# kasirershahartau/tissue_image_processing

Hardware: AMD Instinct MI355X
Metric: frames/sec end-to-end (2048^2, z=30) (higher is better)
Workload: dtype f32(f16x3)

## Files before the change

tissue_image_processing_amd/csrc/tip_core.hip:

```cpp
#include "tip_internal.h"
#include <algorithm>
#include <cmath>
#include <cstdlib>
#include <map>
#include <mutex>

namespace tip {

static thread_local Ctx *g_ctx = nullptr;
static thread_local int g_requested_device = 0;

static int ctx_create(int device)
{
    Ctx *c = new Ctx();
    c->device = device;
    hipError_t e = hipSetDevice(device);
    if (e != hipSuccess) {
        c->err = std::string("hipSetDevice failed: ") + hipGetErrorString(e);
        g_ctx = c;
        return TIP_ERR_HIP;
    }
    {
        const char *pr = getenv("TIP_STREAM_PRIORITY");
        int lo = 0, hi = 0;
        if (pr && hipDeviceGetStreamPriorityRange(&lo, &hi) == hipSuccess && (strcmp(pr, "low") == 0 || strcmp(pr, "high") == 0))
            e = hipStreamCreateWithPriority(&c->stream, hipStreamNonBlocking, strcmp(pr, "low") == 0 ? lo : hi);
        else
            e = hipStreamCreateWithFlags(&c->stream, hipStreamNonBlocking);
    }
    if (e != hipSuccess) {
        c->err = std::string("hipStreamCreate failed: ") + hipGetErrorString(e);
        c->stream = nullptr;
        g_ctx = c;
        return TIP_ERR_HIP;
    }
    g_ctx = c;
    return TIP_OK;
}

Ctx &ctx()
{
    if (!g_ctx) ctx_create(g_requested_device);
    return *g_ctx;
}

int fail(int code, const char *fmt, ...)
{
    char buf[1024];
    va_list ap;
    va_start(ap, fmt);
    vsnprintf(buf, sizeof buf, fmt, ap);
    va_end(ap);
    ctx().err = buf;
    return code;
}

int launch_check(const char *what)
{
    hipError_t e = hipGetLastError();
    if (e != hipSuccess) return fail(TIP_ERR_HIP, "launch %s: %s", what, hipGetErrorString(e));
    return TIP_OK;
}

void *ws_alloc(size_t bytes)
{
    Ctx &c = ctx();
    bytes = (bytes + 255) & ~(size_t)255;
    int best = -1;
    for (size_t i = 0; i < c.pool.size(); i++)
        if (!c.pool[i].used && c.pool[i].bytes >= bytes && (best < 0 || c.pool[i].bytes < c.pool[best].bytes))
            best = (int)i;
    if (best >= 0 && c.pool[best].bytes <= 2 * bytes + (1 << 20)) {
        c.pool[best].used = true;
        return c.pool[best].p;
    }
    void *p = nullptr;
    hipError_t e = hipMalloc(&p, bytes);
    if (e != hipSuccess) {
        for (auto &b : c.pool)
            if (!b.used && b.p) { (void)hipFree(b.p); b.p = nullptr; b.bytes = 0; }
        e = hipMalloc(&p, bytes);
        if (e != hipSuccess) {
            fail(TIP_ERR_NOMEM, "hipMalloc(%zu) failed: %s", bytes, hipGetErrorString(e));
            return nullptr;
        }
    }
    c.pool.push_back({p, bytes, true});
    return p;
}

void *pinned_scratch(size_t bytes)
{
    Ctx &c = ctx();
    if (c.pin_bytes >= bytes && c.pin_buf) return c.pin_buf;
    if (c.pin_buf) { (void)hipHostFree(c.pin_buf); c.pin_buf = nullptr; c.pin_bytes = 0; }
    const size_t want = bytes + (bytes >> 2) + 4096;
    void *p = nullptr;
    if (hipHostMalloc(&p, want, hipHostMallocDefault) != hipSuccess) {
        (void)hipGetLastError();
        fail(TIP_ERR_NOMEM, "hipHostMalloc(%zu) failed", want);
        return nullptr;
    }
    c.pin_buf = p;
    c.pin_bytes = want;
    return p;
}

void ws_free(void *p)
{
    Ctx &c = ctx();
    for (auto &b : c.pool)
        if (b.p == p) { b.used = false; return; }
}

void prof_begin(const char *name)
{
    Ctx &c = ctx();
    if (!c.prof) return;
    ProfRec r;
    r.name = name;
    if (c.free_events.size() >= 2) {
        r.e0 = c.free_events.back(); c.free_events.pop_back();
        r.e1 = c.free_events.back(); c.free_events.pop_back();
    } else {
        (void)hipEventCreate(&r.e0);
        (void)hipEventCreate(&r.e1);
    }
    (void)hipEventRecord(r.e0, c.stream);
    c.recs.push_back(r);
}

void prof_end()
{
    Ctx &c = ctx();
    if (!c.prof) return;
    (void)hipEventRecord(c.recs.back().e1, c.stream);
}

namespace {
Tuning g_tuning;
std::once_flag g_tuning_once;
std::mutex g_tuning_mu;

bool tuning_assign(Tuning &t, const char *name, const char *value)
{
    const Tuning def;
    const bool unset = !value || !*value;
    auto flag = [&](int &field, int dflt) { field = unset ? dflt : (strcmp(value, "0") != 0 ? 1 : 0); };
    auto num = [&](int &field, int dflt) { field = unset ? dflt : atoi(value); };
    auto pair = [&](int &a, int &b, int da, int db) {
        a = da; b = db;
        if (!unset) sscanf(value, "%d,%d", &a, &b);
    };
    const std::string n(name ? name : "");
    if (n == "TIP_WS_TIES") {
        if (unset) t.ws_ties = def.ws_ties;
        else t.ws_ties = (!strcmp(value, "fast") || !strcmp(value, "0")) ? 0 : 1;
    }
    else if (n == "TIP_WS_OPEN") pair(t.ws_open_a, t.ws_open_b, def.ws_open_a, def.ws_open_b);
    else if (n == "TIP_WS_NO_SKIP") flag(t.ws_no_skip, 0);
    else if (n == "TIP_WS_DEBUG") flag(t.ws_debug, 0);
    else if (n == "TIP_WS_NO_ENDGAME") flag(t.ws_no_endgame, 0);
    else if (n == "TIP_WS_NO_WIDE") flag(t.ws_no_wide, 0);
    else if (n == "TIP_PROJECT_GENERIC") flag(t.project_generic, 0);
    else if (n == "TIP_PROJECT_UNFUSED_PREBLUR") flag(t.project_unfused_preblur, 0);
    else if (n == "TIP_PROJECT_UNFUSED_MASK") flag(t.project_unfused_mask, 0);
    else if (n == "TIP_PROJECT_EXACT_SCORE") flag(t.project_exact_score, 0);
    else if (n == "TIP_PROJECT_DEBUG") flag(t.project_debug, 0);
    else if (n == "TIP_UNET_TILE8") num(t.unet_tile8, def.unet_tile8);
    else if (n == "TIP_UF_ONE_LEVEL") flag(t.uf_one_level, 0);
    else if (n == "TIP_UNET_SPB") num(t.unet_spb, def.unet_spb);
    else if (n == "TIP_UNET_MFMA") { num(t.unet_mfma, def.unet_mfma); if (t.unet_mfma != 32) t.unet_mfma = 16; }
    else if (n == "TIP_UNET_XCD_MAP") flag(t.unet_xcd_map, 1);
    else if (n == "TIP_UNET_FIRST") {
        if (unset || !strcmp(value, "mfma")) t.unet_first_mfma = def.unet_first_mfma;
        else t.unet_first_mfma = !strcmp(value, "valu") ? 0 : std::max(atoi(value), 0);
    }
    else if (n == "TIP_UNET_TAIL_UNFUSED") flag(t.unet_tail_unfused, 0);
    else if (n == "TIP_MB_SMALL") num(t.mb_small, def.mb_small);
    else if (n == "TIP_MB_BATCH") num(t.mb_batch, def.mb_batch);
    else return false;
    return true;
}

const char *const TUNING_NAMES[] = {"TIP_WS_TIES", "TIP_WS_OPEN", "TIP_WS_NO_SKIP", "TIP_WS_DEBUG", "TIP_WS_NO_ENDGAME", "TIP_WS_NO_WIDE",
                                    "TIP_PROJECT_GENERIC", "TIP_PROJECT_UNFUSED_PREBLUR", "TIP_PROJECT_UNFUSED_MASK",
                                    "TIP_PROJECT_EXACT_SCORE", "TIP_PROJECT_DEBUG", "TIP_UNET_TILE8", "TIP_UNET_TAIL_UNFUSED", "TIP_UNET_XCD_MAP", "TIP_UNET_SPB", "TIP_UNET_MFMA", "TIP_UNET_FIRST", "TIP_UF_ONE_LEVEL", "TIP_MB_SMALL", "TIP_MB_BATCH"};

void tuning_from_env()
{
    for (const char *name : TUNING_NAMES)
        if (const char *e = getenv(name)) tuning_assign(g_tuning, name, e);
}
}

const Tuning &tuning()
{
    std::call_once(g_tuning_once, tuning_from_env);
    return g_tuning;
}

int make_taps(Taps &t, const double *w, int n)
{
    if (n <= 0 || n > 255 || !(n & 1)) return fail(TIP_ERR_ARG, "tap count %d must be odd and <= 255", n);
    for (int i = 1; i <= n / 2; i++)
        if (fabs(w[n / 2 + i] - w[n / 2 - i]) > 2.220446049250313e-16)
            return fail(TIP_ERR_UNSUPPORTED, "only symmetric kernels (scipy's symmetric correlate1d branch)");
    memset(&t, 0, sizeof t);
    for (int i = 0; i < n; i++) t.w[i] = w[i];
    t.n = n;
    return TIP_OK;
}

static double np_pairwise_sum(const double *a, long n)
{
    if (n < 8) {
        double r = 0.0;
        for (long i = 0; i < n; i++) r += a[i];
        return r;
    } else if (n <= 128) {
        double r[8];
        long i;
        for (i = 0; i < 8; i++) r[i] = a[i];
        for (i = 8; i < n - (n % 8); i += 8)
            for (int k = 0; k < 8; k++) r[k] += a[i + k];
        double res = ((r[0] + r[1]) + (r[2] + r[3])) + ((r[4] + r[5]) + (r[6] + r[7]));
        for (; i < n; i++) res += a[i];
        return res;
    }
    long n2 = n / 2;
    n2 -= n2 % 8;
    return np_pairwise_sum(a, n2) + np_pairwise_sum(a + n2, n - n2);
}

int libm_taps(double sigma, double truncate, double *w, int cap)
{
    long radius = (long)(truncate * sigma + 0.5);
    long n = 2 * radius + 1;
    if (n > cap) return -1;
    double s2 = sigma * sigma;
    for (long i = 0; i < n; i++) {
        double x = (double)(i - radius);
        w[i] = exp(-0.5 / s2 * (x * x));
    }
    double sum = np_pairwise_sum(w, n);
    for (long i = 0; i < n; i++) w[i] = w[i] / sum;
    return (int)n;
}

}

using namespace tip;

extern "C" {

int tip_version(void) { return 100; }

int tip_device_count(void)
{
    int n = 0;
    if (hipGetDeviceCount(&n) != hipSuccess) return 0;
    return n;
}

int tip_init(int device)
{
    if (g_ctx) {
        if (g_ctx->device == device && g_ctx->stream) return TIP_OK;
        tip_shutdown();
    }
    g_requested_device = device;
    int rc = ctx_create(device);
    return rc;
}

int tip_shutdown(void)
{
    if (!g_ctx) return TIP_OK;
    Ctx *c = g_ctx;
    if (c->stream) (void)hipStreamSynchronize(c->stream);
    for (auto &b : c->pool)
        if (b.p) (void)hipFree(b.p);
    for (auto &r : c->recs) { (void)hipEventDestroy(r.e0); (void)hipEventDestroy(r.e1); }
    for (auto &e : c->free_events) (void)hipEventDestroy(e);
    if (c->edge_event) (void)hipEventDestroy(c->edge_event);
    if (c->prep_ws) (void)hipFree(c->prep_ws);
    if (c->unet_status) (void)hipFree(c->unet_status);
    if (c->unet_status_host) (void)hipHostFree(c->unet_status_host);
    if (c->pin_buf) (void)hipHostFree(c->pin_buf);
    if (c->stream) (void)hipStreamDestroy(c->stream);
    delete c;
    g_ctx = nullptr;
    return TIP_OK;
}

int tip_last_error(char *buf, size_t n)
{
    if (!buf || !n) return TIP_ERR_ARG;
    const std::string &e = ctx().err;
    snprintf(buf, n, "%s", e.c_str());
    return TIP_OK;
}

int tip_malloc(void **dptr, size_t bytes)
{
    if (!dptr) return fail(TIP_ERR_ARG, "tip_malloc: null out pointer");
    Ctx &c = ctx();
    if (!c.stream) return TIP_ERR_HIP;
    TIP_HIP(hipMalloc(dptr, bytes ? bytes : 16));
    return TIP_OK;
}

int tip_free(void *dptr)
{
    if (!dptr) return TIP_OK;
    Ctx &c = ctx();
    if (c.stream) TIP_HIP(hipStreamSynchronize(c.stream));
    TIP_HIP(hipFree(dptr));
    return TIP_OK;
}

int tip_memcpy_h2d(void *dst, const void *src, size_t bytes)
{
    Ctx &c = ctx();
    if (!c.stream) return TIP_ERR_HIP;
    TIP_HIP(hipMemcpyAsync(dst, src, bytes, hipMemcpyHostToDevice, c.stream));
    TIP_HIP(hipStreamSynchronize(c.stream));
    return TIP_OK;
}

int tip_memcpy_d2h(void *dst, const void *src, size_t bytes)
{
    Ctx &c = ctx();
    if (!c.stream) return TIP_ERR_HIP;
    TIP_HIP(hipMemcpyAsync(dst, src, bytes, hipMemcpyDeviceToHost, c.stream));
    TIP_HIP(hipStreamSynchronize(c.stream));
    return TIP_OK;
}

int tip_memcpy_d2d(void *dst, const void *src, size_t bytes)
{
    Ctx &c = ctx();
    if (!c.stream) return TIP_ERR_HIP;
    prof_begin("memcpy_d2d");
    const hipError_t e = hipMemcpyAsync(dst, src, bytes, hipMemcpyDeviceToDevice, c.stream);
    prof_end();
    TIP_HIP(e);
    return TIP_OK;
}

int tip_memcpy2d_d2d(void *dst, size_t dst_pitch, const void *src, size_t src_pitch, size_t width_bytes, size_t height)
{
    Ctx &c = ctx();
    if (!c.stream) return TIP_ERR_HIP;
    if (!dst || !src || width_bytes > dst_pitch || width_bytes > src_pitch) return fail(TIP_ERR_ARG, "tip_memcpy2d_d2d: bad arguments");
    if (width_bytes == 0 || height == 0) return TIP_OK;
    TIP_HIP(hipMemcpy2DAsync(dst, dst_pitch, src, src_pitch, width_bytes, height, hipMemcpyDeviceToDevice, c.stream));
    return TIP_OK;
}

int tip_memset(void *dst, int value, size_t bytes)
{
    Ctx &c = ctx();
    if (!c.stream) return TIP_ERR_HIP;
    TIP_HIP(hipMemsetAsync(dst, value, bytes, c.stream));
    return TIP_OK;
}

int tip_sync(void)
{
    Ctx &c = ctx();
    if (!c.stream) return TIP_ERR_HIP;
    TIP_HIP(hipStreamSynchronize(c.stream));
    return TIP_OK;
}

int tip_pointer_device(const void *p)
{
    hipPointerAttribute_t a;
    if (!p || hipPointerGetAttributes(&a, p) != hipSuccess) { (void)hipGetLastError(); return TIP_ERR_ARG; }
    if (a.type != hipMemoryTypeDevice) return TIP_ERR_ARG;
    return a.device;
}

int tip_wait_stream(void *stream)
{
    Ctx &c = ctx();
    if (!c.stream) return TIP_ERR_HIP;
    if (!c.edge_event) TIP_HIP(hipEventCreateWithFlags(&c.edge_event, hipEventDisableTiming));
    TIP_HIP(hipEventRecord(c.edge_event, (hipStream_t)stream));
    TIP_HIP(hipStreamWaitEvent(c.stream, c.edge_event, 0));
    return TIP_OK;
}

int tip_stream_wait_tip(void *stream)
{
    Ctx &c = ctx();
    if (!c.stream) return TIP_ERR_HIP;
    if (!c.edge_event) TIP_HIP(hipEventCreateWithFlags(&c.edge_event, hipEventDisableTiming));
    TIP_HIP(hipEventRecord(c.edge_event, c.stream));
    TIP_HIP(hipStreamWaitEvent((hipStream_t)stream, c.edge_event, 0));
    return TIP_OK;
}

int tip_prof_enable(int on)
{
    ctx().prof = on != 0;
    return TIP_OK;
}

int tip_prof_reset(void)
{
    Ctx &c = ctx();
    if (c.stream) (void)hipStreamSynchronize(c.stream);
    for (auto &r : c.recs) { c.free_events.push_back(r.e0); c.free_events.push_back(r.e1); }
    c.recs.clear();
    return TIP_OK;
}

int tip_prof_report(char *buf, size_t n)
{
    Ctx &c = ctx();
    if (c.stream) (void)hipStreamSynchronize(c.stream);
    std::map<std::string, std::pair<long, double>> agg;
    std::vector<std::string> order;
    for (auto &r : c.recs) {
        float ms = 0.f;
        if (hipEventElapsedTime(&ms, r.e0, r.e1) != hipSuccess) ms = 0.f;
        auto it = agg.find(r.name);
        if (it == agg.end()) { agg[r.name] = {1, (double)ms}; order.push_back(r.name); }
        else { it->second.first++; it->second.second += ms; }
    }
    std::string s;
    char line[256];
    for (auto &k : order) {
        snprintf(line, sizeof line, "%s %ld %.6f\n", k.c_str(), agg[k].first, agg[k].second);
        s += line;
    }
    if (buf && n) snprintf(buf, n, "%s", s.c_str());
    return (int)s.size() + 1;
}

int tip_set_tuning(const char *name, const char *value)
{
    (void)tuning();
    std::lock_guard<std::mutex> lock(g_tuning_mu);
    if (!tuning_assign(g_tuning, name, value)) return fail(TIP_ERR_ARG, "tip_set_tuning: unknown name %s", name ? name : "(null)");
    return TIP_OK;
}

int tip_gaussian_taps(double sigma, double truncate, double *taps, int cap)
{
    if (!taps || sigma <= 0) return fail(TIP_ERR_ARG, "tip_gaussian_taps: bad arguments");
    int n = libm_taps(sigma, truncate, taps, cap);
    if (n < 0) return fail(TIP_ERR_OVERFLOW, "tip_gaussian_taps: capacity %d too small", cap);
    return n;
}

}
```

tissue_image_processing_amd/csrc/tip_corr.h:

```cpp
#pragma once
#include "tip_internal.h"
#include <type_traits>

namespace tip {

template <typename T>
struct LoadPlain {
    const T *p;
    long sz, sy;
    __device__ __forceinline__ double operator()(int z, int y, int x) const { return (double)p[z * sz + y * sy + x]; }
};

__device__ __forceinline__ int clampi(int v, int lo, int hi) { return v < lo ? lo : (v > hi ? hi : v); }

template <int R, typename At, typename W>
__device__ __forceinline__ double tap_sum(At at, const W &w)
{
    double tmp = at(R) * w[R];
#pragma unroll
    for (int d = R; d >= 1; --d) tmp += (at(R - d) + at(R + d)) * w[R - d];
    return tmp;
}
template <typename At, typename W>
__device__ __forceinline__ double tap_sum(int r, At at, const W &w)
{
    double tmp = at(r) * w[r];
    for (int d = r; d >= 1; --d) tmp += (at(r - d) + at(r + d)) * w[r - d];
    return tmp;
}

struct TapsDev {
    const double *w;
    int n;
};

template <int FIRST = 0, typename F>
static inline int with_axis(int axis, F &&f)
{
    if constexpr (FIRST == 0)
        if (axis == 0) return f(std::integral_constant<int, 0>{});
    if (axis == 1) return f(std::integral_constant<int, 1>{});
    return f(std::integral_constant<int, 2>{});
}

template <typename T, int AXIS, typename Load, typename TapSrc = Taps>
__global__ void __launch_bounds__(256) k_corr_generic(Load in, T *__restrict__ out, int Z, int Y, int X, TapSrc taps)
{
    const int x = blockIdx.x * blockDim.x + threadIdx.x;
    const int y = blockIdx.y;
    const int z = blockIdx.z;
    if (x >= X) return;
    const int r = taps.n >> 1;
    const int len = AXIS == 0 ? Z : (AXIS == 1 ? Y : X);
    const int c = AXIS == 0 ? z : (AXIS == 1 ? y : x);
    auto at = [&](int j) -> double {
        const int i = clampi(c - r + j, 0, len - 1);
        return AXIS == 0 ? in(i, y, x) : (AXIS == 1 ? in(z, i, x) : in(z, y, i));
    };
    out[((long)z * Y + y) * X + x] = (T)tap_sum(r, at, taps.w);
}

template <int AXIS, int NW>
__device__ __forceinline__ void stage_tile(float *tile, const float *__restrict__ src, int npos, int first, int l0, int Y, int X,
                                           int lane, int wave)
{
    constexpr int LS = AXIS == 1 ? 64 : 65;
    if (AXIS == 1) {
        constexpr int UL = 8;
        const int xx = min(l0 + lane, X - 1);
        for (int pb = wave; pb < npos; pb += NW * UL) {
            float v[UL];
#pragma unroll
            for (int u = 0; u < UL; ++u) v[u] = src[(long)clampi(first + pb + u * NW, 0, Y - 1) * X + xx];
#pragma unroll
            for (int u = 0; u < UL; ++u)
                if (pb + u * NW < npos) tile[(pb + u * NW) * LS + lane] = v[u];
        }
    } else {
        for (int l = wave; l < 64; l += 2 * NW) {
            float v[2][8];
#pragma unroll
            for (int h = 0; h < 2; ++h) {
                const int yy = min(l0 + l + h * NW, Y - 1);
#pragma unroll
                for (int u = 0; u < 8; ++u) v[h][u] = src[(long)yy * X + clampi(first + lane + 64 * u, 0, X - 1)];
            }
#pragma unroll
            for (int h = 0; h < 2; ++h)
#pragma unroll
                for (int u = 0; u < 8; ++u)
                    if (lane + 64 * u < npos && l + h * NW < 64) tile[(lane + 64 * u) * LS + l + h * NW] = v[h][u];
        }
    }
}

template <int AXIS, int TO, int R>
__global__ void __launch_bounds__(256) k_corr_long_f32(const float *__restrict__ in, float *__restrict__ out,
                                                       int Z, int Y, int X, Taps taps)
{
    extern __shared__ __attribute__((aligned(16))) float tile[];
    constexpr int LS = AXIS == 1 ? 64 : 65;
    const int r = taps.n >> 1;
    const int npos = TO + 2 * r;
    const int lane = threadIdx.x & 63;
    const int wave = threadIdx.x >> 6;
    const int z = blockIdx.z;
    const int len = AXIS == 1 ? Y : X;
    const int nlines = AXIS == 1 ? X : Y;
    const int p0 = blockIdx.y * TO;
    const int l0 = blockIdx.x * 64;
    const float *src = in + (long)z * Y * X;
    float *dst = out + (long)z * Y * X;

    stage_tile<AXIS, 4>(tile, src, npos, p0 - r, l0, Y, X, lane, wave);
    __syncthreads();

    const int line = l0 + lane;
    constexpr int PER_WAVE = TO / 4;
    for (int g = 0; g < PER_WAVE / R; ++g) {
        const int o0 = wave * PER_WAVE + g * R;
        if (p0 + o0 >= len) break;
        const float *ctr = tile + (r + o0) * LS + lane;
        double acc[R], L[R], Rr[R];
        const double wc = taps.w[r];
#pragma unroll
        for (int i = 0; i < R; ++i) {
            acc[i] = (double)ctr[i * LS] * wc;
            L[i] = (double)ctr[(i - r) * LS];
            Rr[i] = (double)ctr[(i + r) * LS];
        }
#pragma unroll 8
        for (int d = r; d >= 1; --d) {
            const double w = taps.w[r - d];
#pragma unroll
            for (int i = 0; i < R; ++i) acc[i] += (L[i] + Rr[i]) * w;
#pragma unroll
            for (int i = 0; i < R - 1; ++i) L[i] = L[i + 1];
            L[R - 1] = (double)ctr[(R - 1 - (d - 1)) * LS];
#pragma unroll
            for (int i = R - 1; i > 0; --i) Rr[i] = Rr[i - 1];
            Rr[0] = (double)ctr[(d - 1) * LS];
        }
        if (line < nlines) {
            if (AXIS == 1) {
#pragma unroll
                for (int i = 0; i < R; ++i) {
                    const int yy = p0 + o0 + i;
                    if (yy < Y) dst[(long)yy * X + line] = (float)acc[i];
                }
            } else {
#pragma unroll
                for (int i = 0; i < R; ++i) {
                    const int xx = p0 + o0 + i;
                    if (xx < X) dst[(long)line * X + xx] = (float)acc[i];
                }
            }
        }
    }
}

}
```

tissue_image_processing_amd/csrc/tip_corr_f16.h:

```cpp
#pragma once
#include "tip_corr.h"
#include "tip_unet_conv.h"

namespace tip {

constexpr int HF_TO = 256, HF_LN = 32, HF_NW = 4;
typedef float hf_f32x4 __attribute__((ext_vector_type(4)));

struct HfScale {
    float s, inv;
};
__device__ __forceinline__ HfScale hf_scale(const float *clip_p95, const int *clip_has)
{
    const float c = (clip_has && *clip_has && *clip_p95 > 0.f) ? *clip_p95 : 1.f;
    const int e = min(max((int)((__float_as_uint(c) >> 23) & 0xffu) - 127, -60), 100);
    HfScale h;
    h.s = __uint_as_float((unsigned)(127 + 13 - e) << 23);
    h.inv = __uint_as_float((unsigned)(127 - 13 + e - 17) << 23);
    return h;
}

template <int AXIS, int R8>
__global__ void __launch_bounds__(HF_NW * 64, 2) k_corr_long_f16(const float *__restrict__ in, float *__restrict__ out, int Z, int Y, int X,
                                                                  TapsF taps, const float *__restrict__ clip_p95, const int *__restrict__ clip_has,
                                                                  int *__restrict__ range_flag, int tiles_ln, int tiles_pos, int xcd_bands)
{
    constexpr int r = 8 * R8, NPOS = HF_TO + 2 * r, S = R8 + 2;
    constexpr int PCH = (NPOS / 8) | 1, PITCH = PCH * 8;
    constexpr int WROWS = 2 * S + 3;
    extern __shared__ __attribute__((aligned(16))) unsigned char hf_smem[];
    _Float16 *sB_hi = reinterpret_cast<_Float16 *>(hf_smem), *sB_lo = sB_hi + HF_LN * PITCH;
    uint4 *sW_hi = reinterpret_cast<uint4 *>(sB_lo + HF_LN * PITCH), *sW_lo = sW_hi + WROWS * 8;
    const int tid = threadIdx.x, lane = tid & 63, wave = __builtin_amdgcn_readfirstlane(tid >> 6);
    const int z = blockIdx.y;
    int lx, py;
    if (AXIS == 2 && xcd_bands) {
        const int b = blockIdx.x, k = b & 7, j = b >> 3;
        py = j % tiles_pos;
        lx = k + 8 * (j / tiles_pos);
    } else {
        lx = blockIdx.x % tiles_ln;
        py = blockIdx.x / tiles_ln;
    }
    const int p0 = py * HF_TO, l0 = lx * HF_LN;
    const long P = (long)Y * X;
    const float *src = in + (long)z * P;
    const HfScale sc = hf_scale(clip_p95, clip_has);

    for (int idx = tid; idx < WROWS * 8; idx += HF_NW * 64) {
        const int up = (idx >> 3) - 3, c = idx & 7;
        f16x8 hi, lo;
#pragma unroll
        for (int e = 0; e < 8; ++e) {
            const int d = 8 * up - c + e, ad = d - r < 0 ? r - d : d - r;
            const float w = (d >= 0 && d <= 2 * r) ? taps.w[r - ad] * 131072.f : 0.f;
            hi[e] = (_Float16)w;
            lo[e] = (_Float16)((w - (float)hi[e]) * 2048.f);
        }
        sW_hi[idx] = __builtin_bit_cast(uint4, hi);
        sW_lo[idx] = __builtin_bit_cast(uint4, lo);
    }
    float vmax = 0.f;
    auto split8 = [&](const float (&v)[8], int line, int g) {
        f16x8 hi, lo;
#pragma unroll
        for (int e = 0; e < 8; ++e) {
            const float vs = v[e] * sc.s;
            vmax = fmax_raw(vmax, vs);
            hi[e] = (_Float16)vs;
            lo[e] = (_Float16)__builtin_fmaf(vs - (float)hi[e], 2048.f, fminf(vs * 1.329227995784916e36f, 5.9604644775390625e-8f));
        }
        *reinterpret_cast<uint4 *>(sB_hi + line * PITCH + 8 * g) = __builtin_bit_cast(uint4, hi);
        *reinterpret_cast<uint4 *>(sB_lo + line * PITCH + 8 * g) = __builtin_bit_cast(uint4, lo);
    };
    constexpr int NG = NPOS / 8;
    if (AXIS == 2) {
        constexpr int NIT = (HF_LN * NG + HF_NW * 64 - 1) / (HF_NW * 64);
        hf_f32x4 ld[NIT][2];
        const bool vec = (X & 3) == 0;
        constexpr int DL = (HF_NW * 64) / NG, DG = (HF_NW * 64) - DL * NG;
        const int line_0 = tid / NG, g_0 = tid - line_0 * NG;
        int uline[NIT], ug[NIT];
        {
            int line = line_0, g = g_0;
#pragma unroll
            for (int it = 0; it < NIT; ++it) {
                uline[it] = line;
                ug[it] = g;
                line += DL;
                g += DG;
                if (g >= NG) { g -= NG; ++line; }
            }
        }
#pragma unroll
        for (int it = 0; it < NIT; ++it) {
            const int line = uline[it], g = ug[it];
            const float *row = src + (long)min(l0 + min(line, HF_LN - 1), Y - 1) * X;
            const int x0 = p0 - r + 8 * g;
            if (vec && x0 >= 0 && x0 + 8 <= X) {
                ld[it][0] = *reinterpret_cast<const hf_f32x4 *>(row + x0);
                ld[it][1] = *reinterpret_cast<const hf_f32x4 *>(row + x0 + 4);
            } else {
                ld[it][0] = hf_f32x4{row[clampi(x0, 0, X - 1)], row[clampi(x0 + 1, 0, X - 1)], row[clampi(x0 + 2, 0, X - 1)], row[clampi(x0 + 3, 0, X - 1)]};
                ld[it][1] = hf_f32x4{row[clampi(x0 + 4, 0, X - 1)], row[clampi(x0 + 5, 0, X - 1)], row[clampi(x0 + 6, 0, X - 1)], row[clampi(x0 + 7, 0, X - 1)]};
            }
        }
#pragma unroll
        for (int it = 0; it < NIT; ++it) {
            const int line = uline[it], g = ug[it];
            if (line < HF_LN) {
                const float v[8] = {ld[it][0][0], ld[it][0][1], ld[it][0][2], ld[it][0][3], ld[it][1][0], ld[it][1][1], ld[it][1][2], ld[it][1][3]};
                split8(v, line, g);
            }
        }
    } else {
        constexpr int NIT = (NG * (HF_LN / 4) + HF_NW * 64 - 1) / (HF_NW * 64);
        hf_f32x4 ld[NIT][8];
        const int lq = tid & 7;
        const int xq = l0 + 4 * lq;
        const bool vec = (X & 3) == 0 && xq + 4 <= X;
        if (vec) {
#pragma unroll
            for (int it = 0; it < NIT; ++it) {
                const int g = min(it * (HF_NW * 8) + (tid >> 3), NG - 1), y0 = p0 - r + 8 * g;
#pragma unroll
                for (int e = 0; e < 8; ++e) ld[it][e] = *reinterpret_cast<const hf_f32x4 *>(src + (long)clampi(y0 + e, 0, Y - 1) * X + xq);
            }
        } else {
#pragma unroll
            for (int it = 0; it < NIT; ++it) {
                const int g = min(it * (HF_NW * 8) + (tid >> 3), NG - 1), y0 = p0 - r + 8 * g;
#pragma unroll
                for (int e = 0; e < 8; ++e) {
                    const float *row = src + (long)clampi(y0 + e, 0, Y - 1) * X;
                    ld[it][e] = hf_f32x4{row[min(xq, X - 1)], row[min(xq + 1, X - 1)], row[min(xq + 2, X - 1)], row[min(xq + 3, X - 1)]};
                }
            }
        }
#pragma unroll
        for (int it = 0; it < NIT; ++it) {
            const int g = it * (HF_NW * 8) + (tid >> 3);
            if (g < NG) {
                float v[8];
#pragma unroll
                for (int e = 0; e < 8; ++e) v[e] = ld[it][e].x;
                split8(v, 4 * lq, g);
#pragma unroll
                for (int e = 0; e < 8; ++e) v[e] = ld[it][e].y;
                split8(v, 4 * lq + 1, g);
#pragma unroll
                for (int e = 0; e < 8; ++e) v[e] = ld[it][e].z;
                split8(v, 4 * lq + 2, g);
#pragma unroll
                for (int e = 0; e < 8; ++e) v[e] = ld[it][e].w;
                split8(v, 4 * lq + 3, g);
            }
        }
    }
    if (!(vmax < 40000.f)) atomicOr(range_flag, 8);
    __syncthreads();

    const int i = lane & 31, h = lane >> 5;
    const int len = AXIS == 1 ? Y : X;
    if (p0 + wave * 64 >= len) return;
    const _Float16 *bh = sB_hi + i * PITCH + wave * 64 + 8 * h, *bl = sB_lo + i * PITCH + wave * 64 + 8 * h;
    const int wrow0 = (h - (i >> 3) + 3) * 8 + (i & 7);
    f32x16 thh[2], tm[2], ahh[2], am[2];
#pragma unroll
    for (int t = 0; t < 2; ++t)
#pragma unroll
        for (int q = 0; q < 16; ++q) { thh[t][q] = 0.f; tm[t][q] = 0.f; ahh[t][q] = 0.f; am[t][q] = 0.f; }
    uint4 fh[3], fl[3];
    auto mm = [](const uint4 &wf, const uint4 &sf, const f32x16 &c) -> f32x16 {
        if (AXIS == 1) return __builtin_amdgcn_mfma_f32_32x32x16_f16(__builtin_bit_cast(f16x8, wf), __builtin_bit_cast(f16x8, sf), c, 0, 0, 0);
        return __builtin_amdgcn_mfma_f32_32x32x16_f16(__builtin_bit_cast(f16x8, sf), __builtin_bit_cast(f16x8, wf), c, 0, 0, 0);
    };
    auto flush = [&](int t) {
#pragma unroll
        for (int q = 0; q < 16; q += 2) {
            f32x2 x = f32x2{thh[t][q], thh[t][q + 1]} + f32x2{ahh[t][q], ahh[t][q + 1]};
            f32x2 y = f32x2{tm[t][q], tm[t][q + 1]} + f32x2{am[t][q], am[t][q + 1]};
            asm volatile("" : "+v"(x), "+v"(y));
            thh[t][q] = x[0]; thh[t][q + 1] = x[1];
            tm[t][q] = y[0]; tm[t][q + 1] = y[1];
            ahh[t][q] = 0.f; ahh[t][q + 1] = 0.f;
            am[t][q] = 0.f; am[t][q + 1] = 0.f;
        }
    };
#pragma unroll
    for (int s = 0; s < S + 2; ++s) {
        const uint4 sh = *reinterpret_cast<const uint4 *>(bh + 16 * s), sl = *reinterpret_cast<const uint4 *>(bl + 16 * s);
        if (s < S) {
            fh[s % 3] = sW_hi[wrow0 + 16 * s];
            fl[s % 3] = sW_lo[wrow0 + 16 * s];
            ahh[0] = mm(fh[s % 3], sh, ahh[0]);
            am[0] = mm(fh[s % 3], sl, am[0]);
            am[0] = mm(fl[s % 3], sh, am[0]);
            if ((s & 1) == 1 || s == S - 1) flush(0);
        }
        if (s >= 2) {
            const int k = (s - 2) % 3;
            ahh[1] = mm(fh[k], sh, ahh[1]);
            am[1] = mm(fh[k], sl, am[1]);
            am[1] = mm(fl[k], sh, am[1]);
            if (((s - 2) & 1) == 1 || s == S + 1) flush(1);
        }
        __builtin_amdgcn_sched_barrier(0);
    }
    float *dst = out + (long)z * P;
#pragma unroll
    for (int t = 0; t < 2; ++t) {
        const int o0 = p0 + wave * 64 + 32 * t;
#pragma unroll
        for (int q = 0; q < 16; ++q) {
            const int rr = (q & 3) + 8 * (q >> 2) + 4 * h;
            const float val = __builtin_fmaf(tm[t][q], 4.8828125e-4f, thh[t][q]) * sc.inv;
            if (AXIS == 1) {
                const int yy = o0 + rr, xx = l0 + i;
                if (yy < Y && xx < X) dst[(long)yy * X + xx] = val;
            } else {
                const int yy = l0 + rr, xx = o0 + i;
                if (yy < Y && xx < X) dst[(long)yy * X + xx] = val;
            }
        }
    }
}

}
```

tissue_image_processing_amd/csrc/tip_internal.h:

```cpp
#pragma once
#include <hip/hip_runtime.h>
#include <cstdarg>
#include <cstdint>
#include <cstdio>
#include <cstring>
#include <string>
#include <vector>
#include "../../include/tissue_hip.h"

namespace tip {

struct ProfRec { const char *name; hipEvent_t e0, e1; };

struct Ctx {
    int device = -1;
    hipStream_t stream = nullptr;
    std::string err;
    struct Block { void *p; size_t bytes; bool used; };
    std::vector<Block> pool;
    int last_ws_labels = 0;
    long last_ws_other = 0;
    hipEvent_t edge_event = nullptr;
    void *prep_ws = nullptr;
    unsigned *unet_status = nullptr;
    int *unet_status_host = nullptr;
    void *pin_buf = nullptr;
    size_t pin_bytes = 0;
    bool prof = false;
    std::vector<ProfRec> recs;
    std::vector<hipEvent_t> free_events;
};

Ctx &ctx();
int fail(int code, const char *fmt, ...);
int launch_check(const char *what);
void *ws_alloc(size_t bytes);
void *pinned_scratch(size_t bytes);
void ws_free(void *p);

struct WsGuard {
    std::vector<void *> ptrs;
    template <typename T> T *get(size_t count) {
        void *p = ws_alloc(count * sizeof(T) ? count * sizeof(T) : 16);
        if (p) ptrs.push_back(p);
        return (T *)p;
    }
    ~WsGuard() { for (void *p : ptrs) ws_free(p); }
};

struct Staging {
    WsGuard ws;
    int rc = TIP_OK;
    struct Out { void *host; const void *dev; size_t bytes; };
    std::vector<Out> outs;

    bool hip(hipError_t e, const char *what)
    {
        if (e != hipSuccess && !rc) rc = fail(TIP_ERR_HIP, "%s failed: %s", what, hipGetErrorString(e));
        return !rc;
    }
    template <typename T> T *scratch(size_t count)
    {
        if (rc) return nullptr;
        T *d = ws.get<T>(count);
        if (!d) rc = TIP_ERR_NOMEM;
        return d;
    }
    template <typename T> T *in(const T *host, size_t count)
    {
        T *d = host ? scratch<T>(count) : nullptr;
        if (d && count) hip(hipMemcpyAsync(d, host, count * sizeof(T), hipMemcpyHostToDevice, ctx().stream), "hipMemcpyAsync (upload)");
        return d;
    }
    template <typename T> T *out(T *host, size_t count, bool zero = false)
    {
        T *d = host ? scratch<T>(count) : nullptr;
        if (d && zero && count) hip(hipMemsetAsync(d, 0, count * sizeof(T), ctx().stream), "hipMemsetAsync");
        if (d) outs.push_back({host, d, count * sizeof(T)});
        return d;
    }
    template <typename T> void set_count(const T *dev, size_t count)
    {
        for (Out &o : outs)
            if (o.dev == dev && count * sizeof(T) < o.bytes) o.bytes = count * sizeof(T);
    }
    int finish()
    {
        for (const Out &o : outs)
            if (o.bytes && !hip(hipMemcpyAsync(o.host, o.dev, o.bytes, hipMemcpyDeviceToHost, ctx().stream), "hipMemcpyAsync (download)")) break;
        if (!rc) hip(hipStreamSynchronize(ctx().stream), "hipStreamSynchronize");
        return rc;
    }
};

void prof_begin(const char *name);
void prof_end();

struct Tuning {
    int ws_ties = 1;
    int ws_open_a = -1, ws_open_b = -1;
    int ws_no_skip = 0;
    int ws_debug = 0;
    int ws_no_endgame = 0, ws_no_wide = 0;
    int project_generic = 0, project_unfused_preblur = 0, project_unfused_mask = 0;
    int project_exact_score = 0, project_debug = 0;
    int unet_tail_unfused = 0;
    int unet_xcd_map = 1;
    int unet_spb = 3;
    int unet_mfma = 32;
    int unet_first_mfma = 1;
    int uf_one_level = 0;
    int mb_small = -1;
    int mb_batch = -1;
    int unet_tile8 = -1;
};
const Tuning &tuning();

#define TIP_HIP(call)                                                                             \
    do {                                                                                          \
        hipError_t e__ = (call);                                                                  \
        if (e__ != hipSuccess)                                                                    \
            return tip::fail(TIP_ERR_HIP, "%s failed: %s (%s:%d)", #call, hipGetErrorString(e__), \
                             __FILE__, __LINE__);                                                 \
    } while (0)

#define TIP_LAUNCH(name, kernel, grid, block, shmem, ...)                                  \
    do {                                                                                   \
        tip::prof_begin(name);                                                             \
        hipLaunchKernelGGL(kernel, grid, block, shmem, tip::ctx().stream, __VA_ARGS__);    \
        tip::prof_end();                                                                   \
        hipError_t e__ = hipGetLastError();                                                \
        if (e__ != hipSuccess)                                                             \
            return tip::fail(TIP_ERR_HIP, "launch %s: %s", name, hipGetErrorString(e__));  \
    } while (0)

static inline int cdiv(long a, long b) { return (int)((a + b - 1) / b); }

struct Taps {
    double w[256];
    int n;
};
struct TapsF {
    float w[256];
    int n;
};

int make_taps(Taps &t, const double *w, int n);
int libm_taps(double sigma, double truncate, double *w, int cap);
int correlate1d_dev(const void *in, void *out, int dtype, int Z, int Y, int X, int axis, const Taps &t, int force);

constexpr int OF_F64_AS_U16 = 5;
int optical_flow_tvl1_dev(const void *ref, const void *mov, int dtype, int y, int x, float attachment, float tightness,
                          int num_warp, int num_iter, double tol, float *flow_out, int32_t *warps_host, int cap);

int exclusive_scan_i32(const int *in, int *out, long n, int *total_dev);
int scan_i32_dev(const int32_t *in, int32_t *out, int n);

int regionprops_dev(const int32_t *labels, const double *intensity, int Y, int X, int n, int64_t *area, int64_t *bbox4, int64_t *sumy,
                    int64_t *sumx, int64_t *pc3, double *isum);
int order_stats_dev(const int32_t *labels, const double *img, long n, int nlab, long long *rank, const long long *rank0, double *lo,
                    double *hi);
int gaussian3d_dev(const void *in, void *out, int dtype, int Z, int Y, int X, const double *tz, int nz, const double *ty, int ny,
                   const double *tx, int nx);
int rankfilter2d_dev(const void *in, void *out, int dtype, int Y, int X, int ky, int kx, int fp, int border, int is_max);
int watershed_dev(const double *img, int32_t *labels, int Y, int X, int wsl, int32_t *flags_host);

template <typename Key, typename F>
__device__ __forceinline__ void wave_combine(bool active, Key key, F f)
{
    unsigned long long todo = __ballot(active);
    const int lane = threadIdx.x & 63;
    while (todo) {
        const int leader = __ffsll((long long)todo) - 1;
        const Key lk = __shfl(key, leader, 64);
        const unsigned long long same = __ballot(active && key == lk) & todo;
        if (lane == leader) f(lk, __popcll(same));
        todo &= ~same;
    }
}

}
```

tissue_image_processing_amd/csrc/tip_project.hip:

```cpp
#include "tip_slide.h"
#include "tip_preblur.h"
#include "tip_corr.h"
#include "tip_corr_f16.h"
#include "tip_manifold.h"
#include "tip_project_binned.h"
#include <algorithm>
#include <atomic>
#include <cstdlib>

namespace tip {

struct ClipInfo {
    double p95d;
    float p95;
    int has;
};

template <typename T>
__device__ __forceinline__ T wave_inclusive_scan(T v, int lane)
{
    for (int d = 1; d < 64; d <<= 1) {
        const T o = __shfl_up(v, d, 64);
        if (lane >= d) v += o;
    }
    return v;
}

constexpr int HIST_PER_BLOCK = 57344;
__device__ __forceinline__ void hist_clear(unsigned int *h)
{
    for (int i = threadIdx.x; i < 32768; i += 1024) h[i] = 0;
    __syncthreads();
}
__device__ __forceinline__ void hist_bump(unsigned int *h, int val) { atomicAdd(&h[val >> 1], 1u << (16 * (val & 1))); }
__device__ __forceinline__ void hist_flush_all(const unsigned int *h, unsigned long long *__restrict__ hist)
{
    for (int i = threadIdx.x; i < 32768; i += 1024) {
        const unsigned int c = h[i];
        if (c & 0xffffu) atomicAdd(&hist[2 * i], (unsigned long long)(c & 0xffffu));
        if (c >> 16) atomicAdd(&hist[2 * i + 1], (unsigned long long)(c >> 16));
    }
}

__global__ void __launch_bounds__(1024) k_hist_u16(const uint16_t *__restrict__ in, long n, int airy,
                                                   unsigned long long *__restrict__ hist)
{
    __shared__ unsigned int h[32768];
    hist_clear(h);
    const long nchunks = (n + HIST_PER_BLOCK - 1) / HIST_PER_BLOCK;
    for (long chunk = blockIdx.x; chunk < nchunks; chunk += gridDim.x) {
        const long base = chunk * HIST_PER_BLOCK;
        constexpr int TRIPS = HIST_PER_BLOCK / (1024 * 8);
        if (base + HIST_PER_BLOCK <= n && ((((uintptr_t)(in + base)) & 15) == 0)) {
            uint4 v[TRIPS];
#pragma unroll
            for (int k = 0; k < TRIPS; ++k) v[k] = *reinterpret_cast<const uint4 *>(in + base + ((long)k * 1024 + threadIdx.x) * 8);
#pragma unroll
            for (int k = 0; k < TRIPS; ++k) {
                const unsigned int w[4] = {v[k].x, v[k].y, v[k].z, v[k].w};
#pragma unroll
                for (int j = 0; j < 4; ++j) {
#pragma unroll
                    for (int s = 0; s < 2; ++s) hist_bump(h, airy_offset((int)((w[j] >> (16 * s)) & 0xffffu), airy));
                }
            }
        } else {
            for (int k = 0; k < TRIPS; ++k) {
                const long i0 = base + ((long)k * 1024 + threadIdx.x) * 8;
                for (int j = 0; j < 8; ++j)
                    if (i0 + j < n) hist_bump(h, airy_offset((int)in[i0 + j], airy));
            }
        }
        __syncthreads();
        if (chunk + gridDim.x < nchunks) {
            for (int i = threadIdx.x; i < 32768; i += 1024) {
                unsigned int c = h[i];
                if ((c & 0xffffu) >= 8192u) { atomicAdd(&hist[2 * i], (unsigned long long)(c & 0xffffu)); c &= 0xffff0000u; h[i] = c; }
                if ((c >> 16) >= 8192u) { atomicAdd(&hist[2 * i + 1], (unsigned long long)(c >> 16)); h[i] = c & 0xffffu; }
            }
            __syncthreads();
        }
    }
    hist_flush_all(h, hist);
}

__global__ void __launch_bounds__(1024) k_hist_u16_box(const uint16_t *__restrict__ in, int Y, int X, int z0, int y0, int x0, int bz,
                                                       int by, int bx, int airy, unsigned long long *__restrict__ hist)
{
    __shared__ unsigned int h[32768];
    hist_clear(h);
    const long n = (long)bz * by * bx;
    const long base = (long)blockIdx.x * HIST_PER_BLOCK;
    for (int k = 0; k < HIST_PER_BLOCK / 1024; ++k) {
        const long i = base + (long)k * 1024 + threadIdx.x;
        if (i < n) {
            const int x = (int)(i % bx), y = (int)((i / bx) % by), z = (int)(i / ((long)bx * by));
            hist_bump(h, airy_offset((int)in[((long)(z0 + z) * Y + (y0 + y)) * X + (x0 + x)], airy));
        }
    }
    __syncthreads();
    hist_flush_all(h, hist);
}

__global__ void __launch_bounds__(1024) k_percentile95(const unsigned long long *__restrict__ hist, ClipInfo *out, int with_zero)
{
    __shared__ unsigned long long wave_tot[16];
    __shared__ unsigned long long s_n;
    __shared__ int s_chunk[2];
    __shared__ unsigned long long s_before[2];
    __shared__ int s_val[2];
    const int t = threadIdx.x, lane = t & 63, wave = t >> 6;
    unsigned long long s = 0;
    for (int b = t * 64; b < t * 64 + 64; ++b)
        if (b > 0 || with_zero) s += hist[b];
    unsigned long long inc = wave_inclusive_scan(s, lane);
    if (lane == 63) wave_tot[wave] = inc;
    __syncthreads();
    unsigned long long base = 0;
    for (int w = 0; w < wave; ++w) base += wave_tot[w];
    inc += base;
    if (t == 1023) s_n = inc;
    __syncthreads();
    const unsigned long long n = s_n;
    if (n == 0) {
        if (t == 0) { out->has = 0; out->p95 = 0.f; out->p95d = 0.0; }
        return;
    }
    const double quant = 95.0 / 100.0;
    const double virt = (double)(n - 1) * quant;
    const double fl = floor(virt);
    const double gamma = virt - fl;
    long long prev = (long long)fl;
    if (prev < 0) prev = 0;
    if (prev > (long long)n - 1) prev = (long long)n - 1;
    long long next = prev + 1;
    if (next > (long long)n - 1) next = (long long)n - 1;
    const unsigned long long exc = inc - s;
    if (s > 0) {
        if (exc <= (unsigned long long)prev && (unsigned long long)prev < inc) { s_chunk[0] = t; s_before[0] = exc; }
        if (exc <= (unsigned long long)next && (unsigned long long)next < inc) { s_chunk[1] = t; s_before[1] = exc; }
    }
    __syncthreads();
    if (wave < 2) {
        const unsigned long long k = (unsigned long long)(wave == 0 ? prev : next) - s_before[wave];
        const int b = s_chunk[wave] * 64 + lane;
        const unsigned long long ci = wave_inclusive_scan((b > 0 || with_zero) ? hist[b] : 0ULL, lane);
        const unsigned long long hit = __ballot(ci > k);
        if (lane == 0) s_val[wave] = hit ? s_chunk[wave] * 64 + (__ffsll((long long)hit) - 1) : 65535;
    }
    __syncthreads();
    if (t != 0) return;
    const float lo = (float)s_val[0], hi = (float)s_val[1];
    const double diff = (double)(hi - lo);
    double res = (double)lo + diff * gamma;
    if (gamma >= 0.5) res = (double)hi - diff * (1.0 - gamma);
    out->p95d = res;
    out->p95 = (float)res;
    out->has = 1;
}

struct LoadU16Clip {
    const uint16_t *p;
    long sz, sy;
    int airy;
    const ClipInfo *clip;
    __device__ __forceinline__ double operator()(int z, int y, int x) const
    {
        return (double)raw_sample(p[z * sz + y * sy + x], airy, clip->has != 0, clip->p95);
    }
};

__device__ __forceinline__ void emit_zmaps(long p, int plane, int Z, int min_z, int atoh_shift, int32_t *__restrict__ zsel,
                                           int32_t *__restrict__ zsel_atoh, int64_t *__restrict__ zmap, int *__restrict__ err)
{
    const int cz = min_z + plane;
    if (zmap) zmap[p] = cz;
    int ca = cz;
    if (atoh_shift != 0) {
        ca = cz + atoh_shift;
        ca = ca < 0 ? 0 : (ca > Z ? Z : ca);
    }
    if (cz >= Z || ca >= Z) {
        atomicOr(err, 1);
        zsel[p] = cz >= Z ? Z - 1 : cz;
        zsel_atoh[p] = ca >= Z ? Z - 1 : ca;
        return;
    }
    zsel[p] = cz;
    zsel_atoh[p] = ca;
}

__global__ void __launch_bounds__(256) k_argmax_z(const float *__restrict__ score, int Z, long P, int min_z,
                                                  int atoh_shift, int32_t *__restrict__ zsel,
                                                  int32_t *__restrict__ zsel_atoh, int64_t *__restrict__ zmap,
                                                  int *__restrict__ err)
{
    const long p = (long)blockIdx.x * blockDim.x + threadIdx.x;
    if (p >= P) return;
    float best = score[p];
    int bi = 0;
    for (int z = 1; z < Z; ++z) {
        const float s = score[(long)z * P + p];
        if (s > best) { best = s; bi = z; }
    }
    emit_zmaps(p, bi, Z, min_z, atoh_shift, zsel, zsel_atoh, zmap, err);
}

__global__ void k_identity(float *out, int n)
{
    const int i = blockIdx.x * blockDim.x + threadIdx.x;
    if (i < n * n) out[i] = (i / n == i % n) ? 1.f : 0.f;
}

struct LoadMaskTable {
    const float *T;
    const int32_t *zsel;
    int Zs;
    long X;
    __device__ __forceinline__ double operator()(int z, int y, int x) const
    {
        return (double)T[z * Zs + zsel[(long)y * X + x]];
    }
};

template <int MAXC>
__global__ void __launch_bounds__(256) k_xpass_wmax(const float *__restrict__ ymask, const uint16_t *__restrict__ img,
                                                    int C, int Zfull, int zlo, int Zs, int Y, int X, int airy,
                                                    unsigned chan_mask, Taps taps, double *__restrict__ proj)
{
    const int x = blockIdx.x * blockDim.x + threadIdx.x;
    const int y = blockIdx.y;
    if (x >= X) return;
    const int r = taps.n >> 1;
    const long P = (long)Y * X;
    float mx[MAXC];
#pragma unroll
    for (int c = 0; c < MAXC; ++c) mx[c] = 0.f;
    for (int z = 0; z < Zs; ++z) {
        const float *row = ymask + (long)z * P + (long)y * X;
        const float m = (float)tap_sum(r, [&](int j) { return (double)row[clampi(x - r + j, 0, X - 1)]; }, taps.w);
#pragma unroll
        for (int c = 0; c < MAXC; ++c) {
            if (c < C && ((chan_mask >> c) & 1u)) {
                const float v = airy_offset((float)img[((long)c * Zfull + zlo + z) * P + (long)y * X + x], airy);
                const float pr = v * m;
                mx[c] = z == 0 ? pr : (pr > mx[c] ? pr : mx[c]);
            }
        }
    }
#pragma unroll
    for (int c = 0; c < MAXC; ++c)
        if (c < C && ((chan_mask >> c) & 1u)) proj[(long)c * P + (long)y * X + x] = (double)mx[c];
}

constexpr int MASK_R = 8, MASK_W = 2 * MASK_R + 1, MASK_ZR = 4;
constexpr int FT_Y = 16, FT_X = 128, FT_W = FT_X + 2 * MASK_R, FT_H = FT_Y + 2 * MASK_R;
template <int MAXC>
__global__ void __launch_bounds__(256) k_mask_wmax_fused(const float *__restrict__ table, const int32_t *__restrict__ zsel,
                                                         const uint16_t *__restrict__ img, int C, int Zfull, int zlo, int Zs, int Y,
                                                         int X, int airy, unsigned chan_mask, Taps taps, double *__restrict__ proj)
{
    extern __shared__ float sT[];
    __shared__ unsigned char zs[FT_H][FT_W];
    __shared__ unsigned char cmin[FT_Y][FT_W], cmax[FT_Y][FT_W];
    __shared__ __attribute__((aligned(16))) float ybuf[2][FT_Y][FT_W];
    __shared__ int s_lo, s_hi;
    const int t = threadIdx.x;
    const int x0 = blockIdx.x * FT_X, y0 = blockIdx.y * FT_Y;
    const long P = (long)Y * X;
    for (int i = t; i < Zs * Zs; i += 256) sT[i] = table[i];
    for (int i = t; i < FT_H * FT_W; i += 256) {
        const int r = i / FT_W, c = i - r * FT_W;
        zs[r][c] = (unsigned char)zsel[(long)clampi(y0 - MASK_R + r, 0, Y - 1) * X + clampi(x0 - MASK_R + c, 0, X - 1)];
    }
    if (t == 0) { s_lo = Zs; s_hi = -1; }
    __syncthreads();
    int lo = Zs, hi = -1;
    for (int i = t; i < FT_Y * FT_W; i += 256) {
        const int r = i / FT_W, c = i - r * FT_W;
        int a = zs[r][c], b = a;
#pragma unroll
        for (int k = 1; k < MASK_W; ++k) { const int v = zs[r + k][c]; a = min(a, v); b = max(b, v); }
        cmin[r][c] = (unsigned char)a; cmax[r][c] = (unsigned char)b;
        lo = min(lo, a); hi = max(hi, b);
    }
    for (int d = 32; d >= 1; d >>= 1) { lo = min(lo, __shfl_xor(lo, d, 64)); hi = max(hi, __shfl_xor(hi, d, 64)); }
    if ((t & 63) == 0) { atomicMin(&s_lo, lo); atomicMax(&s_hi, hi); }
    __syncthreads();
    const int zaB = max(s_lo - MASK_ZR, 0), zbB = min(s_hi + MASK_ZR, Zs - 1);
    const int ty = t >> 4, cx = (t & 15) * 8;
    const int gy = y0 + ty, gx = x0 + cx;
    const bool live = gy < Y && gx < X;
    int za = Zs, zb = -1;
    if (live) {
        for (int c = cx; c < cx + 8 + 2 * MASK_R; ++c) { za = min(za, (int)cmin[ty][c]); zb = max(zb, (int)cmax[ty][c]); }
        za = max(za - MASK_ZR, 0); zb = min(zb + MASK_ZR, Zs - 1);
    }
    float mx[MAXC][8];
#pragma unroll
    for (int c = 0; c < MAXC; ++c)
#pragma unroll
        for (int k = 0; k < 8; ++k) mx[c][k] = 0.f;
    for (int z = zaB; z <= zbB; ++z) {
        float(*yb)[FT_W] = ybuf[(z - zaB) & 1];
        const float *Tz = sT + z * Zs;
        for (int i = t; i < FT_Y * FT_W; i += 256) {
            const int r = i / FT_W, c = i - r * FT_W;
            float val = 0.f;
            if (z >= (int)cmin[r][c] - MASK_ZR && z <= (int)cmax[r][c] + MASK_ZR)
                val = (float)tap_sum<MASK_R>([&](int j) { return (double)Tz[zs[r + j][c]]; }, taps.w);
            yb[r][c] = val;
        }
        __syncthreads();
        if (live && z >= za && z <= zb) {
            float v[8 + 2 * MASK_R];
#pragma unroll
            for (int i = 0; i < (8 + 2 * MASK_R) / 4; ++i) {
                const float4 f = *reinterpret_cast<const float4 *>(&yb[ty][cx + 4 * i]);
                v[4 * i] = f.x; v[4 * i + 1] = f.y; v[4 * i + 2] = f.z; v[4 * i + 3] = f.w;
            }
            float m[8];
#pragma unroll
            for (int k = 0; k < 8; ++k) m[k] = (float)tap_sum<MASK_R>([&](int j) { return (double)v[k + j]; }, taps.w);
#pragma unroll
            for (int c = 0; c < MAXC; ++c) {
                if (c < C && ((chan_mask >> c) & 1u)) {
                    const uint16_t *ip = img + ((long)c * Zfull + zlo + z) * P + (long)gy * X + gx;
                    unsigned short pix[8];
                    if (gx + 8 <= X && (X & 7) == 0) {
                        const uint4 u = *reinterpret_cast<const uint4 *>(ip);
                        pix[0] = u.x & 0xffff; pix[1] = u.x >> 16; pix[2] = u.y & 0xffff; pix[3] = u.y >> 16;
                        pix[4] = u.z & 0xffff; pix[5] = u.z >> 16; pix[6] = u.w & 0xffff; pix[7] = u.w >> 16;
                    } else {
#pragma unroll
                        for (int k = 0; k < 8; ++k) pix[k] = gx + k < X ? ip[k] : 0;
                    }
#pragma unroll
                    for (int k = 0; k < 8; ++k) {
                        const float pr = airy_offset((float)pix[k], airy) * m[k];
                        mx[c][k] = pr > mx[c][k] ? pr : mx[c][k];
                    }
                }
            }
        }
    }
    if (live) {
#pragma unroll
        for (int c = 0; c < MAXC; ++c)
            if (c < C && ((chan_mask >> c) & 1u))
#pragma unroll
                for (int k = 0; k < 8; ++k)
                    if (gx + k < X) proj[(long)c * P + (long)gy * X + gx + k] = (double)mx[c][k];
    }
}

static int cu_count()
{
    static int cus = 0;
    if (!cus) {
        hipDeviceProp_t prop;
        cus = hipGetDeviceProperties(&prop, ctx().device) == hipSuccess && prop.multiProcessorCount > 0 ? prop.multiProcessorCount : 256;
    }
    return cus;
}

static TapsF taps_f32(const double *w, int n)
{
    TapsF f;
    f.n = n;
    for (int i = 0; i < 256; ++i) f.w[i] = i < n ? (float)w[i] : 0.f;
    return f;
}

template <int AXIS>
static int launch_f16(const float *in, float *out, int Zs, int Y, int X, const TapsF &t, const ClipInfo *clip, int *range_flag)
{
    if (t.n != 241 || !clip || !range_flag) return fail(TIP_ERR_ARG, "f16 score pass: %d taps (241 only) or no clip value / range flag", t.n);
    constexpr int R8 = 15, NPOS = HF_TO + 16 * R8, PITCH = ((NPOS / 8) | 1) * 8, WROWS = 2 * (R8 + 2) + 3;
    const size_t lds = (size_t)2 * HF_LN * PITCH * 2 + (size_t)2 * WROWS * 8 * 16;
    auto k = k_corr_long_f16<AXIS, R8>;
    static std::atomic<unsigned> attr_done[64];
    const int dev = ctx().device >= 0 && ctx().device < 64 ? ctx().device : 0;
    if (!(attr_done[dev].load(std::memory_order_acquire) & (1u << AXIS))) {
        TIP_HIP(hipFuncSetAttribute((const void *)k, hipFuncAttributeMaxDynamicSharedMemorySize, (int)lds));
        attr_done[dev].fetch_or(1u << AXIS, std::memory_order_release);
    }
    const int tiles_ln = cdiv(AXIS == 1 ? X : Y, HF_LN), tiles_pos = cdiv(AXIS == 1 ? Y : X, HF_TO);
    if ((long)tiles_ln * tiles_pos > 0x7fffffffL || Zs > 65535) return fail(TIP_ERR_ARG, "f16 score pass: grid too large");
    const dim3 grid((unsigned)(tiles_ln * tiles_pos), (unsigned)Zs);
    const int xcd_bands = (AXIS == 2 && tiles_ln % 8 == 0) ? 1 : 0;
    TIP_LAUNCH(AXIS == 1 ? "score_fast_y" : "score_fast_x", k, grid, dim3(HF_NW * 64), lds, in, out, Zs, Y, X, t, &clip->p95, &clip->has, range_flag,
               tiles_ln, tiles_pos, xcd_bands);
    return TIP_OK;
}

#define CERT_EPS (96.0f * 5.9604644775390625e-8f)
__device__ __forceinline__ float cert_abs(const ClipInfo *clip)
{
    return (clip && clip->has) ? clip->p95 * 5.684341886080802e-14f + 1e-30f : 1e-30f;
}

__global__ void __launch_bounds__(256) k_argmax_certify(const float *__restrict__ score, int Z, long P, int *__restrict__ best_z,
                                                        int *__restrict__ unc_list, int *__restrict__ unc_count, const ClipInfo *clip)
{
    __shared__ int s_cnt[4], s_base;
    const float dabs = cert_abs(clip);
    const long p0 = ((long)blockIdx.x * blockDim.x + threadIdx.x) * 4;
    const bool vec = p0 + 4 <= P && (P & 3) == 0;
    float b1[4], b2[4];
    int z1[4];
#pragma unroll
    for (int k = 0; k < 4; ++k) { b1[k] = -1.f; b2[k] = -1.f; z1[k] = 0; }
    if (p0 < P) {
        for (int z = 0; z < Z; ++z) {
            float v[4];
            if (vec) {
                const float4 f = *reinterpret_cast<const float4 *>(score + (long)z * P + p0);
                v[0] = f.x; v[1] = f.y; v[2] = f.z; v[3] = f.w;
            } else {
#pragma unroll
                for (int k = 0; k < 4; ++k) v[k] = p0 + k < P ? score[(long)z * P + p0 + k] : 0.f;
            }
#pragma unroll
            for (int k = 0; k < 4; ++k) {
                if (v[k] > b1[k]) { b2[k] = b1[k]; b1[k] = v[k]; z1[k] = z; }
                else if (v[k] > b2[k]) b2[k] = v[k];
            }
        }
    }
    unsigned unc = 0;
#pragma unroll
    for (int k = 0; k < 4; ++k) {
        if (p0 + k >= P) continue;
        best_z[p0 + k] = z1[k];
        const bool certain = (b1[k] == 0.f) || (Z == 1) || (b1[k] * (1.f - CERT_EPS) - dabs > b2[k] * (1.f + CERT_EPS) + dabs);
        if (!certain) unc |= 1u << k;
    }
    const int mine = __popc(unc);
    const int lane = threadIdx.x & 63, wave = threadIdx.x >> 6;
    const int incl = wave_inclusive_scan(mine, lane);
    if (lane == 63) s_cnt[wave] = incl;
    __syncthreads();
    if (threadIdx.x == 0) {
        const int tot = s_cnt[0] + s_cnt[1] + s_cnt[2] + s_cnt[3];
        s_base = tot ? atomicAdd(unc_count, tot) : 0;
    }
    __syncthreads();
    if (mine) {
        int off = s_base + incl - mine;
        for (int w = 0; w < wave; ++w) off += s_cnt[w];
#pragma unroll
        for (int k = 0; k < 4; ++k)
            if ((unc >> k) & 1u) unc_list[off++] = (int)(p0 + k);
    }
}

constexpr int FIX_UL = 16;
__global__ void __launch_bounds__(256) k_argmax_exact_fix(const float *__restrict__ zvol, const float *__restrict__ score, int Z, int Y,
                                                          int X, Taps taps, const int *__restrict__ unc_list,
                                                          const int *__restrict__ unc_count, int *__restrict__ best_z, const ClipInfo *clip)
{
    const float dabs = cert_abs(clip);
    __shared__ float c[256];
    __shared__ float sfast[64];
    __shared__ float sexact[64];
    __shared__ int s_z;
    const int r = taps.n >> 1;
    const int total = *unc_count, xcd = blockIdx.x & 7, per = (total + 7) / 8;
    for (int sl = blockIdx.x >> 3; sl < per; sl += gridDim.x >> 3) {
        const int u = xcd * per + sl;
        if (u >= total) break;
        const int p = unc_list[u];
        const int y = p / X, x = p - y * X;
        const long P = (long)Y * X;
        if (threadIdx.x < Z) sfast[threadIdx.x] = score[(long)threadIdx.x * P + p];
        __syncthreads();
        float smax = sfast[0];
        for (int z = 1; z < Z; ++z) smax = fmaxf(smax, sfast[z]);
        const float thr = smax * (1.f - CERT_EPS) - dabs;
        for (int z = 0; z < Z; ++z) {
            const bool cand = sfast[z] * (1.f + CERT_EPS) + dabs >= thr;
            if (!cand) { if (threadIdx.x == 0) sexact[z] = -1.f; continue; }
            const float *vol = zvol + (long)z * P;
            if (threadIdx.x < 2 * r + 1) {
                const int xx = clampi(x + (int)threadIdx.x - r, 0, X - 1);
                double tmp = (double)vol[(long)y * X + xx] * taps.w[r];
                for (int d0 = r; d0 >= 1; d0 -= FIX_UL) {
                    float a[FIX_UL], b[FIX_UL];
#pragma unroll
                    for (int u = 0; u < FIX_UL; ++u) {
                        const int d = max(d0 - u, 1);
                        a[u] = vol[(long)clampi(y - d, 0, Y - 1) * X + xx];
                        b[u] = vol[(long)clampi(y + d, 0, Y - 1) * X + xx];
                    }
#pragma unroll
                    for (int u = 0; u < FIX_UL; ++u)
                        if (d0 - u >= 1) tmp += ((double)a[u] + (double)b[u]) * taps.w[r - (d0 - u)];
                }
                c[threadIdx.x] = (float)tmp;
            }
            __syncthreads();
            if (threadIdx.x == 0) sexact[z] = (float)tap_sum(r, [&](int j) { return (double)c[j]; }, taps.w);
            __syncthreads();
        }
        if (threadIdx.x == 0) {
            float b = -2.f; int bz = 0;
            for (int z = 0; z < Z; ++z)
                if (sexact[z] > b) { b = sexact[z]; bz = z; }
            best_z[p] = bz;
        }
        __syncthreads();
    }
}

__global__ void __launch_bounds__(256) k_emit_zmaps(const int *__restrict__ best_z, int Z, long P, int min_z, int atoh_shift,
                                                    int32_t *__restrict__ zsel, int32_t *__restrict__ zsel_atoh,
                                                    int64_t *__restrict__ zmap, int *__restrict__ err)
{
    const long p = (long)blockIdx.x * blockDim.x + threadIdx.x;
    if (p >= P) return;
    emit_zmaps(p, best_z[p], Z, min_z, atoh_shift, zsel, zsel_atoh, zmap, err);
}

static int resolve_taps(const double *given, double sigma, int expect, Taps &t)
{
    double buf[256];
    if (!given) {
        int n = libm_taps(sigma, 4.0, buf, 255);
        if (n != expect) return fail(TIP_ERR_ARG, "internal: tap count %d != %d", n, expect);
        given = buf;
    }
    return make_taps(t, given, expect);
}

static int manifold_dev(const float *score, int Zs, int Y, int X, int *bestz, int *err)
{
    Ctx &c = ctx();
    const long P = (long)Y * X, V = (long)Zs * P;
    if (V >= 0xffffffffL || Zs > 144 || Zs < 1) return fail(TIP_ERR_UNSUPPORTED, "build_manifold: stack too large");
    WsGuard ws;
    unsigned long long *key = ws.get<unsigned long long>(1);
    if (!key) return TIP_ERR_NOMEM;
    TIP_HIP(hipMemsetAsync(key, 0, sizeof(unsigned long long), c.stream));
    TIP_HIP(hipMemsetAsync(bestz, 0xff, P * sizeof(int), c.stream));
    TIP_LAUNCH("argmax_first", k_argmax_first_f32, dim3((unsigned)std::min<long>(1024, cdiv(V, 256))), dim3(256), 0, score, V, key);
    int chunk = 1024;
    while (chunk > 64 && (size_t)4 * Zs * chunk > 150000) chunk >>= 1;
    const size_t lds = (size_t)4 * Zs * chunk;
    TIP_HIP(hipFuncSetAttribute((const void *)k_manifold, hipFuncAttributeMaxDynamicSharedMemorySize, (int)lds));
    TIP_LAUNCH("manifold", k_manifold, dim3(1), dim3(MAN_T), lds, score, Zs, Y, X, (const unsigned long long *)key, (volatile int *)bestz,
               chunk, err);
    return TIP_OK;
}

struct ProjJob {
    const uint16_t *czyx, *ref;
    int C, Z, Y, X, zlo, Zs;
    long P, V;
    int min_z, ref_ch, method, bin, airyscan, atoh_shift;
    bool manifold;
    bool ref_unshifted;
    bool fast;
    Taps k05, k1, k2, k30;
    WsGuard ws;
    float *A, *B;
    unsigned long long *hist;
    ClipInfo *clip;
    int32_t *zsel, *zsel_a;
    float *ident, *table;
    int *err;
    double *proj;
    int64_t *zmap;
    hipStream_t stream;
};

static int check_args(const ProjJob &s, int zhi, bool tile)
{
    if (!s.czyx || !s.proj) return fail(TIP_ERR_ARG, "project: null pointer");
    if (s.C < 1 || s.C > 8) return fail(TIP_ERR_ARG, "project: 1..8 channels supported (got %d)", s.C);
    if (s.ref_ch < 0 || s.ref_ch >= s.C) return fail(TIP_ERR_INDEX, "project: reference_channel %d out of range", s.ref_ch);
    if (s.zlo < 0 || zhi > s.Z || zhi <= s.zlo) return fail(TIP_ERR_ARG, "project: bad z range [%d,%d) of %d", s.zlo, zhi, s.Z);
    if (s.Y < 1 || s.X < 1 || s.Y > 65535) return fail(TIP_ERR_ARG, "project: bad frame size %dx%d", s.Y, s.X);
    if (s.manifold && tile) return fail(TIP_ERR_UNSUPPORTED, "project: build_manifold takes whole frames");
    if (s.manifold && (s.V >= 0xffffffffL || s.Zs > 144)) return fail(TIP_ERR_UNSUPPORTED, "project: build_manifold: stack too large");
    return TIP_OK;
}

static int take_workspace(ProjJob &s)
{
    s.A = s.ws.get<float>(s.V), s.B = s.ws.get<float>(s.V);
    s.hist = s.ws.get<unsigned long long>(65536);
    s.clip = s.ws.get<ClipInfo>(1);
    s.zsel = s.ws.get<int32_t>(s.P), s.zsel_a = s.ws.get<int32_t>(s.P);
    s.ident = s.ws.get<float>((size_t)s.Zs * s.Zs), s.table = s.ws.get<float>((size_t)s.Zs * s.Zs);
    s.err = s.ws.get<int>(1);
    if (!s.A || !s.B || !s.hist || !s.clip || !s.zsel || !s.zsel_a || !s.ident || !s.table || !s.err) return TIP_ERR_NOMEM;
    return TIP_OK;
}

static int clip_of_channel(ProjJob &s, const uint16_t *src, int with_zero, ClipInfo *clip)
{
    TIP_HIP(hipMemsetAsync(s.hist, 0, 65536 * sizeof(unsigned long long), s.stream));
    TIP_LAUNCH("hist_u16", k_hist_u16, dim3((unsigned)std::min<long>(cdiv(s.V, HIST_PER_BLOCK), cu_count())), dim3(1024), 0, src, s.V,
               s.airyscan, s.hist);
    TIP_LAUNCH("percentile95", k_percentile95, dim3(1), dim3(1024), 0, (const unsigned long long *)s.hist, clip, with_zero);
    return TIP_OK;
}

static int short_blur(ProjJob &s, const uint16_t *src, ClipInfo *ci)
{
    const int Zs = s.Zs, Y = s.Y, X = s.X;
    if (s.fast && s.bin == 1 && !tuning().project_unfused_preblur) {
        ShortTaps s05, s1;
        for (int i = 0; i < 8; ++i) { s05.w[i] = i < 3 ? s.k05.w[i] : 0.0; s1.w[i] = i < 5 ? s.k1.w[i] : 0.0; }
        TIP_LAUNCH("preblur_fused", k_preblur_fused, dim3(cdiv(X, PB_X), cdiv(Y, PB_Y)), dim3(PB_T), 0, src, s.airyscan,
                   (const float *)&ci->p95, (const int *)&ci->has, s.B, Zs, Y, X, s05, s1);
        return TIP_OK;
    }
    if (s.fast) {
        Src4U16Clip su{src, s.airyscan, &ci->p95, &ci->has};
        TIP_LAUNCH("zpass_u16clip_x4", (k_zpass_r2_x4<Src4U16Clip>), dim3(cdiv(s.P / 4, 256)), dim3(256), 0, su, s.A, Zs, s.P, s.k05);
        TIP_LAUNCH("ypass_slide_r4", (k_ypass_slide<float, 4, 4>), dim3(cdiv(X, 256), cdiv(Y, 36), Zs), dim3(256), 0,
                   (const float *)s.A, s.B, Y, X, s.k1);
        TIP_LAUNCH("xpass_slide_r4", (k_xpass_slide<float, 4>), dim3(cdiv(cdiv(X, 8), 256), Y, Zs), dim3(256), 0, (const float *)s.B,
                   s.A, Y, X, s.k1);
        Src4F32 sf{s.A};
        TIP_LAUNCH("zpass_f32_x4", (k_zpass_r2_x4<Src4F32>), dim3(cdiv(s.P / 4, 256)), dim3(256), 0, sf, s.B, Zs, s.P, s.k05);
        return TIP_OK;
    }
    LoadU16Clip ld{src, s.P, (long)X, s.airyscan, ci};
    dim3 grid(cdiv(X, 256), Y, Zs), block(256);
    TIP_LAUNCH("corr_z_u16clip", (k_corr_generic<float, 0, LoadU16Clip>), grid, block, 0, ld, s.A, Zs, Y, X, s.k05);
    int rc;
    if ((rc = correlate1d_dev(s.A, s.B, 0, Zs, Y, X, 1, s.k1, 0))) return rc;
    if ((rc = correlate1d_dev(s.B, s.A, 0, Zs, Y, X, 2, s.k1, 0))) return rc;
    return correlate1d_dev(s.A, s.B, 0, Zs, Y, X, 0, s.k05, 0);
}

static int score_exact(ProjJob &s)
{
    int rc;
    if ((rc = correlate1d_dev(s.B, s.A, 0, s.Zs, s.Y, s.X, 1, s.k30, 0))) return rc;
    return correlate1d_dev(s.A, s.B, 0, s.Zs, s.Y, s.X, 2, s.k30, 0);
}

static int emit_from_planes(ProjJob &s, const int *bestz, int min_z)
{
    TIP_LAUNCH("emit_zmaps", k_emit_zmaps, dim3(cdiv(s.P, 256)), dim3(256), 0, bestz, s.Zs, s.P, min_z, s.atoh_shift, s.zsel, s.zsel_a,
               s.zmap, s.err);
    return TIP_OK;
}

static int zmaps_binned(ProjJob &s)
{
    const int Zs = s.Zs, Y = s.Y, X = s.X, bin = s.bin, Yb = cdiv(Y, bin), Xb = cdiv(X, bin);
    const long nb = (long)Zs * Yb * Xb;
    float *S1 = s.ws.get<float>(nb);
    int *bestz = s.ws.get<int>(s.P);
    if (!S1 || !bestz) return TIP_ERR_NOMEM;
    int rc;
    if (s.method == 0) {
        if ((rc = score_exact(s))) return rc;
        TIP_LAUNCH("block_mean", (k_block_reduce<false>), dim3(cdiv(nb, 256)), dim3(256), 0, (const float *)s.B, S1, Zs, Y, X, bin, Yb, Xb);
    } else {
        TIP_LAUNCH("block_var", (k_block_reduce<true>), dim3(cdiv(nb, 256)), dim3(256), 0, (const float *)s.A, S1, Zs, Y, X, bin, Yb, Xb);
    }
    if (s.method == 2) {
        const uint16_t *other = s.czyx + ((long)((s.ref_ch + 1) % s.C) * s.Z + s.zlo) * s.P;
        float *S2 = s.ws.get<float>(nb);
        ClipInfo *clip2 = s.ws.get<ClipInfo>(1);
        if (!S2 || !clip2) return TIP_ERR_NOMEM;
        if ((rc = clip_of_channel(s, other, 1, clip2)) || (rc = short_blur(s, other, clip2)) || (rc = score_exact(s))) return rc;
        TIP_LAUNCH("block_mean", (k_block_reduce<false>), dim3(cdiv(nb, 256)), dim3(256), 0, (const float *)s.B, S2, Zs, Y, X, bin, Yb, Xb);
        TIP_LAUNCH("mul_f32", k_mul_f32, dim3(cdiv(nb, 256)), dim3(256), 0, S1, (const float *)S2, nb);
    }
    if (!s.manifold) {
        TIP_LAUNCH("resize_argmax", k_resize_argmax, dim3(cdiv(X, 256), Y), dim3(256), 0, (const float *)S1, Zs, Yb, Xb, Y, X, bestz);
        return emit_from_planes(s, bestz, s.min_z);
    }
    int *bz = s.ws.get<int>((size_t)Yb * Xb);
    if (!bz) return TIP_ERR_NOMEM;
    if ((rc = manifold_dev((const float *)S1, Zs, Yb, Xb, bz, s.err))) return rc;
    TIP_LAUNCH("resize_round_zmaps", k_resize_round_zmaps, dim3(cdiv(X, 256), Y), dim3(256), 0, (const int *)bz, Yb, Xb, Y, X, Zs,
               s.atoh_shift, s.zsel, s.zsel_a, s.zmap, s.err);
    return TIP_OK;
}

static int zmaps_certified(ProjJob &s)
{
    const int Zs = s.Zs, Y = s.Y, X = s.X;
    const long P = s.P;
    float *D = s.ws.get<float>(s.V);
    int *bestz = s.ws.get<int>(P), *unc = s.ws.get<int>(P), *uncn = s.ws.get<int>(1);
    if (!D || !bestz || !unc || !uncn) return TIP_ERR_NOMEM;
    const TapsF f30 = taps_f32(s.k30.w, s.k30.n);
    int rc;
    if ((rc = launch_f16<1>((const float *)s.B, s.A, Zs, Y, X, f30, s.clip, s.err))) return rc;
    if ((rc = launch_f16<2>((const float *)s.A, D, Zs, Y, X, f30, s.clip, s.err))) return rc;
    TIP_HIP(hipMemsetAsync(uncn, 0, sizeof(int), s.stream));
    TIP_LAUNCH("argmax_certify", k_argmax_certify, dim3(cdiv(cdiv(P, 4), 256)), dim3(256), 0, (const float *)D, Zs, P, bestz, unc, uncn,
               (const ClipInfo *)s.clip);
    TIP_LAUNCH("argmax_exact_fix", k_argmax_exact_fix, dim3(8192), dim3(256), 0, (const float *)s.B, (const float *)D, Zs, Y, X,
               s.k30, (const int *)unc, (const int *)uncn, bestz, (const ClipInfo *)s.clip);
    if ((rc = emit_from_planes(s, bestz, s.min_z))) return rc;
    if (tuning().project_debug) {
        int hn = 0, he = 0;
        TIP_HIP(hipMemcpyAsync(&hn, uncn, sizeof(int), hipMemcpyDeviceToHost, s.stream));
        TIP_HIP(hipMemcpyAsync(&he, s.err, sizeof(int), hipMemcpyDeviceToHost, s.stream));
        TIP_HIP(hipStreamSynchronize(s.stream));
        fprintf(stderr, "certified argmax: %d of %ld pixels recomputed exactly\n", hn, P);
        if (he & 8) return fail(TIP_ERR_HIP, "score pass: a sample beyond the clip value's range reached the fp16 tiles");
    }
    return TIP_OK;
}

static int zmaps_full(ProjJob &s)
{
    if (s.fast && s.Zs <= 64 && !s.manifold && !tuning().project_exact_score) return zmaps_certified(s);
    int rc;
    if ((rc = score_exact(s))) return rc;
    if (!s.manifold) {
        TIP_LAUNCH("argmax_z", k_argmax_z, dim3(cdiv(s.P, 256)), dim3(256), 0, s.B, s.Zs, s.P, s.min_z, s.atoh_shift, s.zsel, s.zsel_a,
                   s.zmap, s.err);
        return TIP_OK;
    }
    int *bestz = s.ws.get<int>(s.P);
    if (!bestz) return TIP_ERR_NOMEM;
    if ((rc = manifold_dev((const float *)s.B, s.Zs, s.Y, s.X, bestz, s.err))) return rc;
    return emit_from_planes(s, bestz, 0);
}

template <int MAXC>
static int launch_mask_fused(const ProjJob &s, const int32_t *sel, unsigned cm)
{
    TIP_LAUNCH("mask_wmax_fused", (k_mask_wmax_fused<MAXC>), dim3(cdiv(s.X, FT_X), cdiv(s.Y, FT_Y)), dim3(256),
               (size_t)s.Zs * s.Zs * sizeof(float), (const float *)s.table, sel, s.czyx, s.C, s.Z, s.zlo, s.Zs, s.Y, s.X, s.airyscan, cm,
               s.k2, s.proj);
    return TIP_OK;
}

static int mask_and_project(ProjJob &s)
{
    const int Zs = s.Zs, Y = s.Y, X = s.X, C = s.C;
    TIP_LAUNCH("identity", k_identity, dim3(cdiv((long)Zs * Zs, 256)), dim3(256), 0, s.ident, Zs);
    int rc;
    if ((rc = correlate1d_dev(s.ident, s.table, 0, Zs, Zs, 1, 0, s.k1, 1))) return rc;
    const bool fused = s.fast && Zs <= 64 && !tuning().project_unfused_mask;
    const unsigned all = (1u << C) - 1u;
    for (int pass = 0; pass < (s.atoh_shift != 0 ? 2 : 1); ++pass) {
        const int32_t *sel = pass == 0 ? s.zsel : s.zsel_a;
        const unsigned refbit = s.ref_unshifted ? (1u << s.ref_ch) : 0u;
        const unsigned cm = s.atoh_shift == 0 ? all : (pass == 0 ? refbit : (all & ~refbit));
        if (!cm) continue;
        if (fused) {
            rc = C <= 2 ? launch_mask_fused<2>(s, sel, cm) : C <= 4 ? launch_mask_fused<4>(s, sel, cm) : launch_mask_fused<8>(s, sel, cm);
            if (rc) return rc;
            continue;
        }
        LoadMaskTable ld{s.table, sel, Zs, (long)X};
        dim3 grid(cdiv(X, 256), Y, Zs), block(256);
        TIP_LAUNCH("mask_ypass", (k_corr_generic<float, 1, LoadMaskTable>), grid, block, 0, ld, s.A, Zs, Y, X, s.k2);
        TIP_LAUNCH("xpass_wmax", (k_xpass_wmax<8>), dim3(cdiv(X, 256), Y), dim3(256), 0, s.A, s.czyx, C, s.Z, s.zlo, Zs, Y, X, s.airyscan,
                   cm, s.k2, s.proj);
    }
    return TIP_OK;
}

static int read_err(ProjJob &s)
{
    if (!(s.min_z > 0 || s.atoh_shift > 0 || s.manifold)) return TIP_OK;
    int h = 0;
    TIP_HIP(hipMemcpyAsync(&h, s.err, sizeof(int), hipMemcpyDeviceToHost, s.stream));
    TIP_HIP(hipStreamSynchronize(s.stream));
    if (h & 2) return fail(TIP_ERR_HIP, "build_manifold: a pixel without a visited neighbour (upstream raises TypeError here)");
    if (h & 8) return fail(TIP_ERR_HIP, "score pass: a sample beyond the clip value's range reached the fp16 tiles");
    if (h)
        return fail(TIP_ERR_INDEX, "chosen z index out of bounds for the %d-plane mask (min_z=%d, atoh_shift=%d): "
                                   "the reference raises IndexError here (sp.py:62,68-69)", s.Zs, s.min_z, s.atoh_shift);
    return TIP_OK;
}

int project_dev(const uint16_t *czyx, int C, int Z, int Y, int X, int zlo, int zhi, int min_z, int ref_ch, int method, int bin,
                int airyscan, int atoh_shift, const double *t05, const double *t1, const double *t2,
                const double *t30, double *proj, int64_t *zmap, const unsigned long long *hist_in = nullptr)
{
    ProjJob s;
    s.stream = ctx().stream;
    if (!s.stream) return TIP_ERR_HIP;
    s.czyx = czyx; s.C = C; s.Z = Z; s.Y = Y; s.X = X; s.zlo = zlo; s.Zs = zhi - zlo;
    s.P = (long)Y * X; s.V = (long)s.Zs * s.P;
    s.ref_unshifted = ref_ch >= 0;
    if (ref_ch < 0 && C > 0) ref_ch += C;
    s.min_z = min_z; s.ref_ch = ref_ch; s.bin = bin; s.airyscan = airyscan; s.atoh_shift = atoh_shift;
    s.manifold = (method & TIP_PROJECT_MANIFOLD) != 0;
    s.method = method & ~TIP_PROJECT_MANIFOLD;
    s.fast = (X % 4 == 0) && !tuning().project_generic;
    s.proj = proj; s.zmap = zmap;
    int rc;
    if ((rc = check_args(s, zhi, hist_in != nullptr)) || (rc = resolve_taps(t05, 0.5, 5, s.k05)) || (rc = resolve_taps(t1, 1.0, 9, s.k1)) ||
        (rc = resolve_taps(t2, 2.0, 17, s.k2)) || (rc = resolve_taps(t30, 30.0, 241, s.k30)) || (rc = take_workspace(s)))
        return rc;
    s.ref = czyx + ((long)ref_ch * Z + zlo) * s.P;
    TIP_HIP(hipMemsetAsync(s.err, 0, sizeof(int), s.stream));
    if (hist_in) {
        if (bin > 1 && s.method == 2) return fail(TIP_ERR_UNSUPPORTED, "project: tiles with method multi_channel");
        TIP_LAUNCH("percentile95", k_percentile95, dim3(1), dim3(1024), 0, hist_in, s.clip, 0);
    } else if ((rc = clip_of_channel(s, s.ref, 0, s.clip))) return rc;
    if ((rc = short_blur(s, s.ref, s.clip))) return rc;
    if ((rc = bin > 1 ? zmaps_binned(s) : zmaps_full(s))) return rc;
    if ((rc = mask_and_project(s))) return rc;
    return read_err(s);
}

}

using namespace tip;

extern "C" {

static int project_host(const uint16_t *czyx, int c, int z, int y, int x, int zlo, int zhi, int min_z, int ref_ch, int method,
                        int bin, int airyscan, int atoh_shift, const double *t05, const double *t1, const double *t2,
                        const double *t30, double *proj, int64_t *zmap)
{
    if (!ctx().stream) return TIP_ERR_HIP;
    if (!czyx || !proj) return fail(TIP_ERR_ARG, "tip_project_u16: null pointer");
    if (c < 1 || z < 1 || y < 1 || x < 1) return fail(TIP_ERR_ARG, "tip_project_u16: empty stack");
    const size_t nin = (size_t)c * z * y * x, P = (size_t)y * x;
    Staging st;
    const uint16_t *din = st.in(czyx, nin);
    double *dproj = st.out(proj, (size_t)c * P);
    int64_t *dz = st.out(zmap, P);
    if (st.rc) return st.rc;
    int rc = project_dev(din, c, z, y, x, zlo, zhi, min_z, ref_ch, method, bin, airyscan, atoh_shift, t05, t1, t2, t30, dproj, dz);
    if (rc) return rc;
    return st.finish();
}

static int check_binned(int method, int bin)
{
    if (method >= 0) method &= ~TIP_PROJECT_MANIFOLD;
    if (method < 0 || method > 2) return fail(TIP_ERR_ARG, "projection: method %d (0 max_averages, 1 max_std, 2 multi_channel)", method);
    if (bin < 1 || bin > 128) return fail(TIP_ERR_UNSUPPORTED, "projection: bin_size %d (1..128 supported)", bin);
    return TIP_OK;
}

int tip_project_u16_dev(const uint16_t *czyx, int c, int z, int y, int x, int zlo, int zhi, int min_z, int ref_ch,
                        int airyscan, int atoh_shift, const double *t05, const double *t1, const double *t2,
                        const double *t30, double *proj, int64_t *zmap)
{
    return project_dev(czyx, c, z, y, x, zlo, zhi, min_z, ref_ch, 0, 1, airyscan, atoh_shift, t05, t1, t2, t30, proj, zmap);
}

int tip_project_u16(const uint16_t *czyx, int c, int z, int y, int x, int zlo, int zhi, int min_z, int ref_ch,
                    int airyscan, int atoh_shift, const double *t05, const double *t1, const double *t2,
                    const double *t30, double *proj, int64_t *zmap)
{
    return project_host(czyx, c, z, y, x, zlo, zhi, min_z, ref_ch, 0, 1, airyscan, atoh_shift, t05, t1, t2, t30, proj, zmap);
}

int tip_hist_u16_box_dev(const uint16_t *czyx, int c, int z, int y, int x, int ch, int z0, int z1, int y0, int y1, int x0, int x1,
                         int airyscan, unsigned long long *hist_dev)
{
    Ctx &cx = ctx();
    if (!cx.stream) return TIP_ERR_HIP;
    if (!czyx || !hist_dev) return fail(TIP_ERR_ARG, "tip_hist_u16_box_dev: null pointer");
    if (ch < 0 || ch >= c || z0 < 0 || z1 > z || z1 <= z0 || y0 < 0 || y1 > y || y1 <= y0 || x0 < 0 || x1 > x || x1 <= x0)
        return fail(TIP_ERR_ARG, "tip_hist_u16_box_dev: box outside the (%d,%d,%d,%d) stack", c, z, y, x);
    const long n = (long)(z1 - z0) * (y1 - y0) * (x1 - x0);
    const uint16_t *plane = czyx + (long)ch * z * y * x;
    TIP_LAUNCH("hist_u16_box", k_hist_u16_box, dim3(cdiv(n, HIST_PER_BLOCK)), dim3(1024), 0, plane, y, x, z0, y0, x0, z1 - z0, y1 - y0,
               x1 - x0, airyscan, hist_dev);
    return TIP_OK;
}

int tip_project_u16_hist_dev(const uint16_t *czyx, int c, int z, int y, int x, int zlo, int zhi, int min_z, int ref_ch,
                             int airyscan, int atoh_shift, const double *t05, const double *t1, const double *t2,
                             const double *t30, const unsigned long long *hist_dev, double *proj, int64_t *zmap)
{
    if (!hist_dev) return fail(TIP_ERR_ARG, "tip_project_u16_hist_dev: null histogram");
    return project_dev(czyx, c, z, y, x, zlo, zhi, min_z, ref_ch, 0, 1, airyscan, atoh_shift, t05, t1, t2, t30, proj, zmap, hist_dev);
}

int tip_project_u16_binned_dev(const uint16_t *czyx, int c, int z, int y, int x, int zlo, int zhi, int min_z, int ref_ch,
                               int method, int bin_size, int airyscan, int atoh_shift, const double *t05, const double *t1,
                               const double *t2, const double *t30, double *proj, int64_t *zmap)
{
    int rc = check_binned(method, bin_size);
    if (rc) return rc;
    return project_dev(czyx, c, z, y, x, zlo, zhi, min_z, ref_ch, method, bin_size, airyscan, atoh_shift, t05, t1, t2, t30, proj, zmap);
}

int tip_project_u16_binned(const uint16_t *czyx, int c, int z, int y, int x, int zlo, int zhi, int min_z, int ref_ch,
                           int method, int bin_size, int airyscan, int atoh_shift, const double *t05, const double *t1,
                           const double *t2, const double *t30, double *proj, int64_t *zmap)
{
    int rc = check_binned(method, bin_size);
    if (rc) return rc;
    return project_host(czyx, c, z, y, x, zlo, zhi, min_z, ref_ch, method, bin_size, airyscan, atoh_shift, t05, t1, t2, t30, proj, zmap);
}

__global__ void k_set_clip(ClipInfo *c, float v) { c->has = 1; c->p95 = v; c->p95d = (double)v; }

int tip_score_pass_f16(const float *in, float *out, int z, int y, int x, int axis, const double *taps, int ntaps, float clip, int *flag)
{
    if (!ctx().stream) return TIP_ERR_HIP;
    if (!in || !out || !taps || !flag || z < 1 || y < 1 || x < 1 || (axis != 1 && axis != 2) || ntaps != 241 || !(clip > 0.f))
        return fail(TIP_ERR_ARG, "tip_score_pass_f16: bad arguments (radius 120 only)");
    const size_t V = (size_t)z * y * x;
    Staging st;
    const float *di = st.in(in, V);
    float *dout = st.out(out, V);
    ClipInfo *ci = st.scratch<ClipInfo>(1);
    int *df = st.out(flag, 1, true);
    if (st.rc) return st.rc;
    const TapsF t = taps_f32(taps, ntaps);
    hipLaunchKernelGGL(k_set_clip, dim3(1), dim3(1), 0, ctx().stream, ci, clip);
    int rc = with_axis<1>(axis, [&](auto A) { return launch_f16<decltype(A)::value>(di, dout, z, y, x, t, ci, df); });
    if (rc) return rc;
    return st.finish();
}

__global__ void k_mfma_f16_probe(const float *a, const float *b, const float *c, float *out, int ncase)
{
    const int h = threadIdx.x >> 5;
    for (int t = 0; t < ncase; ++t) {
        f16x8 fa, fb;
        for (int e = 0; e < 8; ++e) { fa[e] = (_Float16)a[t * 16 + 8 * h + e]; fb[e] = (_Float16)b[t * 16 + 8 * h + e]; }
        f32x16 acc;
        for (int q = 0; q < 16; ++q) acc[q] = c[t];
        acc = __builtin_amdgcn_mfma_f32_32x32x16_f16(fa, fb, acc, 0, 0, 0);
        if (threadIdx.x == 0) out[t] = acc[0];
    }
}
int tip_mfma_f16_probe(const float *a, const float *b, const float *cvals, float *out, int ncase)
{
    if (!ctx().stream) return TIP_ERR_HIP;
    if (!a || !b || !cvals || !out || ncase < 1 || ncase > 256) return fail(TIP_ERR_ARG, "tip_mfma_f16_probe: bad arguments");
    Staging st;
    const float *da = st.in(a, (size_t)ncase * 16), *db = st.in(b, (size_t)ncase * 16), *dc = st.in(cvals, (size_t)ncase);
    float *dout = st.out(out, (size_t)ncase);
    if (st.rc) return st.rc;
    hipLaunchKernelGGL(k_mfma_f16_probe, dim3(1), dim3(64), 0, ctx().stream, da, db, dc, dout, ncase);
    return st.finish();
}

int tip_build_manifold_f32(const float *score, int z, int y, int x, int64_t *chosen)
{
    if (!ctx().stream) return TIP_ERR_HIP;
    if (!score || !chosen || z < 1 || y < 1 || x < 1) return fail(TIP_ERR_ARG, "tip_build_manifold_f32: bad arguments");
    const size_t P = (size_t)y * x, V = P * z;
    std::vector<int> hb(P);
    int herr = 0;
    Staging st;
    const float *ds = st.in(score, V);
    int *bz = st.out(hb.data(), P), *err = st.out(&herr, 1, true);
    if (st.rc) return st.rc;
    int rc = manifold_dev(ds, z, y, x, bz, err);
    if (rc) return rc;
    if ((rc = st.finish())) return rc;
    if (herr) return fail(TIP_ERR_HIP, "build_manifold: a pixel without a visited neighbour (upstream raises TypeError here)");
    for (size_t i = 0; i < P; ++i) chosen[i] = hb[i];
    return TIP_OK;
}

}
```

Before: 21.96.

## Fuse z-argmax into x-pass f16 correlation kernel and batch exact fixes by cell

The last separable correlation pass now loops over all z planes inside each block and keeps a per-pixel top-two tracker with candidate plane masks, so it no longer writes the full score volume. The certify kernel reads the compact top-two buffers instead of scanning the volume. The exact-fix kernel groups uncertain pixels in the same 16-wide cell and recomputes only the candidate planes per pixel. This removes a large volume write and re-read, at the cost of register pressure and less parallelism per block in the fused pass.

After: 21.96, median of 2. About the same (-0.0%).

```diff
diff --git a/tissue_image_processing_amd/csrc/tip_core.hip b/tissue_image_processing_amd/csrc/tip_core.hip
--- a/tissue_image_processing_amd/csrc/tip_core.hip
+++ b/tissue_image_processing_amd/csrc/tip_core.hip
@@ -167,6 +167,7 @@
     else if (n == "TIP_PROJECT_UNFUSED_MASK") flag(t.project_unfused_mask, 0);
     else if (n == "TIP_PROJECT_EXACT_SCORE") flag(t.project_exact_score, 0);
     else if (n == "TIP_PROJECT_DEBUG") flag(t.project_debug, 0);
+    else if (n == "TIP_ARGMAX_FUSED") flag(t.argmax_fused, 1);
     else if (n == "TIP_UNET_TILE8") num(t.unet_tile8, def.unet_tile8);
     else if (n == "TIP_UF_ONE_LEVEL") flag(t.uf_one_level, 0);
     else if (n == "TIP_UNET_SPB") num(t.unet_spb, def.unet_spb);
@@ -185,7 +186,7 @@
 
 const char *const TUNING_NAMES[] = {"TIP_WS_TIES", "TIP_WS_OPEN", "TIP_WS_NO_SKIP", "TIP_WS_DEBUG", "TIP_WS_NO_ENDGAME", "TIP_WS_NO_WIDE",
                                     "TIP_PROJECT_GENERIC", "TIP_PROJECT_UNFUSED_PREBLUR", "TIP_PROJECT_UNFUSED_MASK",
-                                    "TIP_PROJECT_EXACT_SCORE", "TIP_PROJECT_DEBUG", "TIP_UNET_TILE8", "TIP_UNET_TAIL_UNFUSED", "TIP_UNET_XCD_MAP", "TIP_UNET_SPB", "TIP_UNET_MFMA", "TIP_UNET_FIRST", "TIP_UF_ONE_LEVEL", "TIP_MB_SMALL", "TIP_MB_BATCH"};
+                                    "TIP_PROJECT_EXACT_SCORE", "TIP_PROJECT_DEBUG", "TIP_ARGMAX_FUSED", "TIP_UNET_TILE8", "TIP_UNET_TAIL_UNFUSED", "TIP_UNET_XCD_MAP", "TIP_UNET_SPB", "TIP_UNET_MFMA", "TIP_UNET_FIRST", "TIP_UF_ONE_LEVEL", "TIP_MB_SMALL", "TIP_MB_BATCH"};
 
 void tuning_from_env()
 {
diff --git a/tissue_image_processing_amd/csrc/tip_corr.h b/tissue_image_processing_amd/csrc/tip_corr.h
--- a/tissue_image_processing_amd/csrc/tip_corr.h
+++ b/tissue_image_processing_amd/csrc/tip_corr.h
@@ -12,6 +12,16 @@
 };
 
 __device__ __forceinline__ int clampi(int v, int lo, int hi) { return v < lo ? lo : (v > hi ? hi : v); }
+
+template <typename T>
+__device__ __forceinline__ T wave_inclusive_scan(T v, int lane)
+{
+    for (int d = 1; d < 64; d <<= 1) {
+        const T o = __shfl_up(v, d, 64);
+        if (lane >= d) v += o;
+    }
+    return v;
+}
 
 template <int R, typename At, typename W>
 __device__ __forceinline__ double tap_sum(At at, const W &w)
diff --git a/tissue_image_processing_amd/csrc/tip_corr_f16.h b/tissue_image_processing_amd/csrc/tip_corr_f16.h
--- a/tissue_image_processing_amd/csrc/tip_corr_f16.h
+++ b/tissue_image_processing_amd/csrc/tip_corr_f16.h
@@ -20,11 +20,49 @@
     return h;
 }
 
-template <int AXIS, int R8>
+#define CERT_EPS (96.0f * 5.9604644775390625e-8f)
+__device__ __forceinline__ float cert_abs(const float *clip_p95, const int *clip_has)
+{
+    return (clip_has && *clip_has) ? *clip_p95 * 5.684341886080802e-14f + 1e-30f : 1e-30f;
+}
+__device__ __forceinline__ bool cert_cand(float s, float smax, float dabs)
+{
+    return s * (1.f + CERT_EPS) + dabs >= smax * (1.f - CERT_EPS) - dabs;
+}
+struct CertTop {
+    float b1, b2;
+    unsigned zz;
+};
+__device__ __forceinline__ CertTop cert_start() { return CertTop{-1.f, -1.f, 0u}; }
+__device__ __forceinline__ void cert_push(CertTop &c, float v, int z, float dabs)
+{
+    const bool g1 = v > c.b1, g2 = v > c.b2;
+    const float below = fminf(c.b2, v), old1 = c.b1;
+    c.b2 = g1 ? c.b1 : (g2 ? v : c.b2);
+    c.b1 = g1 ? v : c.b1;
+    const unsigned zp = c.zz & 0xfffu, more = c.zz & 0x1000u;
+    const unsigned zn = g1 ? (((zp << 6) & 0xfc0u) | (unsigned)z) : (g2 ? ((zp & 0x3fu) | ((unsigned)z << 6)) : zp);
+    const bool keep = !g1 || cert_cand(old1, c.b1, dabs);
+    c.zz = zn | (keep ? more : 0u) | (cert_cand(below, c.b1, dabs) ? 0x1000u : 0u);
+}
+__device__ __forceinline__ int cert_best(const CertTop &c) { return (int)(c.zz & 0x3fu); }
+__device__ __forceinline__ bool cert_certain(const CertTop &c, int Z, float dabs)
+{
+    return (c.b1 == 0.f) || (Z == 1) || (c.b1 * (1.f - CERT_EPS) - dabs > c.b2 * (1.f + CERT_EPS) + dabs);
+}
+__device__ __forceinline__ unsigned long long cert_planes(const CertTop &c, int Z)
+{
+    if (c.zz & 0x1000u) return Z >= 64 ? ~0ULL : (1ULL << Z) - 1ULL;
+    return (1ULL << (c.zz & 0x3fu)) | (1ULL << ((c.zz >> 6) & 0x3fu));
+}
+
+template <int AXIS, int R8, bool ARGMAX = false>
 __global__ void __launch_bounds__(HF_NW * 64, 2) k_corr_long_f16(const float *__restrict__ in, float *__restrict__ out, int Z, int Y, int X,
                                                                   TapsF taps, const float *__restrict__ clip_p95, const int *__restrict__ clip_has,
-                                                                  int *__restrict__ range_flag, int tiles_ln, int tiles_pos, int xcd_bands)
-{
+                                                                  int *__restrict__ range_flag, int tiles_ln, int tiles_pos, int xcd_bands,
+                                                                  float2 *__restrict__ top_b, unsigned *__restrict__ top_z)
+{
+    static_assert(!ARGMAX || AXIS == 2, "the argmax rides on the last pass");
     constexpr int r = 8 * R8, NPOS = HF_TO + 2 * r, S = R8 + 2;
     constexpr int PCH = (NPOS / 8) | 1, PITCH = PCH * 8;
     constexpr int WROWS = 2 * S + 3;
@@ -32,7 +70,6 @@
     _Float16 *sB_hi = reinterpret_cast<_Float16 *>(hf_smem), *sB_lo = sB_hi + HF_LN * PITCH;
     uint4 *sW_hi = reinterpret_cast<uint4 *>(sB_lo + HF_LN * PITCH), *sW_lo = sW_hi + WROWS * 8;
     const int tid = threadIdx.x, lane = tid & 63, wave = __builtin_amdgcn_readfirstlane(tid >> 6);
-    const int z = blockIdx.y;
     int lx, py;
     if (AXIS == 2 && xcd_bands) {
         const int b = blockIdx.x, k = b & 7, j = b >> 3;
@@ -44,7 +81,6 @@
     }
     const int p0 = py * HF_TO, l0 = lx * HF_LN;
     const long P = (long)Y * X;
-    const float *src = in + (long)z * P;
     const HfScale sc = hf_scale(clip_p95, clip_has);
 
     for (int idx = tid; idx < WROWS * 8; idx += HF_NW * 64) {
@@ -60,133 +96,191 @@
         sW_hi[idx] = __builtin_bit_cast(uint4, hi);
         sW_lo[idx] = __builtin_bit_cast(uint4, lo);
     }
-    float vmax = 0.f;
-    auto split8 = [&](const float (&v)[8], int line, int g) {
-        f16x8 hi, lo;
-#pragma unroll
-        for (int e = 0; e < 8; ++e) {
-            const float vs = v[e] * sc.s;
-            vmax = fmax_raw(vmax, vs);
-            hi[e] = (_Float16)vs;
-            lo[e] = (_Float16)__builtin_fmaf(vs - (float)hi[e], 2048.f, fminf(vs * 1.329227995784916e36f, 5.9604644775390625e-8f));
-        }
-        *reinterpret_cast<uint4 *>(sB_hi + line * PITCH + 8 * g) = __builtin_bit_cast(uint4, hi);
-        *reinterpret_cast<uint4 *>(sB_lo + line * PITCH + 8 * g) = __builtin_bit_cast(uint4, lo);
+    auto stage = [&](const float *src) {
+        float vmax = 0.f;
+        auto split8 = [&](const float (&v)[8], int line, int g) {
+            f16x8 hi, lo;
+#pragma unroll
+            for (int e = 0; e < 8; ++e) {
+                const float vs = v[e] * sc.s;
+                vmax = fmax_raw(vmax, vs);
+                hi[e] = (_Float16)vs;
+                lo[e] = (_Float16)__builtin_fmaf(vs - (float)hi[e], 2048.f, fminf(vs * 1.329227995784916e36f, 5.9604644775390625e-8f));
+            }
+            *reinterpret_cast<uint4 *>(sB_hi + line * PITCH + 8 * g) = __builtin_bit_cast(uint4, hi);
+            *reinterpret_cast<uint4 *>(sB_lo + line * PITCH + 8 * g) = __builtin_bit_cast(uint4, lo);
+        };
+        constexpr int NG = NPOS / 8;
+        if (AXIS == 2) {
+            constexpr int NIT = (HF_LN * NG + HF_NW * 64 - 1) / (HF_NW * 64);
+            hf_f32x4 ld[NIT][2];
+            const bool vec = (X & 3) == 0;
+            constexpr int DL = (HF_NW * 64) / NG, DG = (HF_NW * 64) - DL * NG;
+            const int line_0 = tid / NG, g_0 = tid - line_0 * NG;
+            int uline[NIT], ug[NIT];
+            {
+                int line = line_0, g = g_0;
+                if (ARGMAX) asm volatile("" : "+v"(line), "+v"(g));
+#pragma unroll
+                for (int it = 0; it < NIT; ++it) {
+                    uline[it] = line;
+                    ug[it] = g;
+                    line += DL;
+                    g += DG;
+                    if (g >= NG) { g -= NG; ++line; }
+                }
+            }
+#pragma unroll
+            for (int it = 0; it < NIT; ++it) {
+                const int line = uline[it], g = ug[it];
+                const float *row = src + (long)min(l0 + min(line, HF_LN - 1), Y - 1) * X;
+                const int x0 = p0 - r + 8 * g;
+                if (vec && x0 >= 0 && x0 + 8 <= X) {
+                    ld[it][0] = *reinterpret_cast<const hf_f32x4 *>(row + x0);
+                    ld[it][1] = *reinterpret_cast<const hf_f32x4 *>(row + x0 + 4);
+                } else {
+                    ld[it][0] = hf_f32x4{row[clampi(x0, 0, X - 1)], row[clampi(x0 + 1, 0, X - 1)], row[clampi(x0 + 2, 0, X - 1)], row[clampi(x0 + 3, 0, X - 1)]};
+                    ld[it][1] = hf_f32x4{row[clampi(x0 + 4, 0, X - 1)], row[clampi(x0 + 5, 0, X - 1)], row[clampi(x0 + 6, 0, X - 1)], row[clampi(x0 + 7, 0, X - 1)]};
+                }
+            }
+#pragma unroll
+            for (int it = 0; it < NIT; ++it) {
+                const int line = uline[it], g = ug[it];
+                if (line < HF_LN) {
+                    const float v[8] = {ld[it][0][0], ld[it][0][1], ld[it][0][2], ld[it][0][3], ld[it][1][0], ld[it][1][1], ld[it][1][2], ld[it][1][3]};
+                    split8(v, line, g);
+                }
+            }
+        } else {
+            constexpr int NIT = (NG * (HF_LN / 4) + HF_NW * 64 - 1) / (HF_NW * 64);
+            hf_f32x4 ld[NIT][8];
+            const int lq = tid & 7;
+            const int xq = l0 + 4 * lq;
+            const bool vec = (X & 3) == 0 && xq + 4 <= X;
+            if (vec) {
+#pragma unroll
+                for (int it = 0; it < NIT; ++it) {
+                    const int g = min(it * (HF_NW * 8) + (tid >> 3), NG - 1), y0 = p0 - r + 8 * g;
+#pragma unroll
+                    for (int e = 0; e < 8; ++e) ld[it][e] = *reinterpret_cast<const hf_f32x4 *>(src + (long)clampi(y0 + e, 0, Y - 1) * X + xq);
+                }
+            } else {
+#pragma unroll
+                for (int it = 0; it < NIT; ++it) {
+                    const int g = min(it * (HF_NW * 8) + (tid >> 3), NG - 1), y0 = p0 - r + 8 * g;
+#pragma unroll
+                    for (int e = 0; e < 8; ++e) {
+                        const float *row = src + (long)clampi(y0 + e, 0, Y - 1) * X;
+                        ld[it][e] = hf_f32x4{row[min(xq, X - 1)], row[min(xq + 1, X - 1)], row[min(xq + 2, X - 1)], row[min(xq + 3, X - 1)]};
+                    }
+                }
+            }
+#pragma unroll
+            for (int it = 0; it < NIT; ++it) {
+                const int g = it * (HF_NW * 8) + (tid >> 3);
+                if (g < NG) {
+                    float v[8];
+#pragma unroll
+                    for (int e = 0; e < 8; ++e) v[e] = ld[it][e].x;
+                    split8(v, 4 * lq, g);
+#pragma unroll
+                    for (int e = 0; e < 8; ++e) v[e] = ld[it][e].y;
+                    split8(v, 4 * lq + 1, g);
+#pragma unroll
+                    for (int e = 0; e < 8; ++e) v[e] = ld[it][e].z;
+                    split8(v, 4 * lq + 2, g);
+#pragma unroll
+                    for (int e = 0; e < 8; ++e) v[e] = ld[it][e].w;
+                    split8(v, 4 * lq + 3, g);
+                }
+            }
+        }
+        if (!(vmax < 40000.f)) atomicOr(range_flag, 8);
     };
-    constexpr int NG = NPOS / 8;
-    if (AXIS == 2) {
-        constexpr int NIT = (HF_LN * NG + HF_NW * 64 - 1) / (HF_NW * 64);
-        hf_f32x4 ld[NIT][2];
-        const bool vec = (X & 3) == 0;
-        constexpr int DL = (HF_NW * 64) / NG, DG = (HF_NW * 64) - DL * NG;
-        const int line_0 = tid / NG, g_0 = tid - line_0 * NG;
-        int uline[NIT], ug[NIT];
-        {
-            int line = line_0, g = g_0;
-#pragma unroll
-            for (int it = 0; it < NIT; ++it) {
-                uline[it] = line;
-                ug[it] = g;
-                line += DL;
-                g += DG;
-                if (g >= NG) { g -= NG; ++line; }
-            }
-        }
-#pragma unroll
-        for (int it = 0; it < NIT; ++it) {
-            const int line = uline[it], g = ug[it];
-            const float *row = src + (long)min(l0 + min(line, HF_LN - 1), Y - 1) * X;
-            const int x0 = p0 - r + 8 * g;
-            if (vec && x0 >= 0 && x0 + 8 <= X) {
-                ld[it][0] = *reinterpret_cast<const hf_f32x4 *>(row + x0);
-                ld[it][1] = *reinterpret_cast<const hf_f32x4 *>(row + x0 + 4);
-            } else {
-                ld[it][0] = hf_f32x4{row[clampi(x0, 0, X - 1)], row[clampi(x0 + 1, 0, X - 1)], row[clampi(x0 + 2, 0, X - 1)], row[clampi(x0 + 3, 0, X - 1)]};
-                ld[it][1] = hf_f32x4{row[clampi(x0 + 4, 0, X - 1)], row[clampi(x0 + 5, 0, X - 1)], row[clampi(x0 + 6, 0, X - 1)], row[clampi(x0 + 7, 0, X - 1)]};
-            }
-        }
-#pragma unroll
-        for (int it = 0; it < NIT; ++it) {
-            const int line = uline[it], g = ug[it];
-            if (line < HF_LN) {
-                const float v[8] = {ld[it][0][0], ld[it][0][1], ld[it][0][2], ld[it][0][3], ld[it][1][0], ld[it][1][1], ld[it][1][2], ld[it][1][3]};
-                split8(v, line, g);
-            }
-        }
-    } else {
-        constexpr int NIT = (NG * (HF_LN / 4) + HF_NW * 64 - 1) / (HF_NW * 64);
-        hf_f32x4 ld[NIT][8];
-        const int lq = tid & 7;
-        const int xq = l0 + 4 * lq;
-        const bool vec = (X & 3) == 0 && xq + 4 <= X;
-        if (vec) {
-#pragma unroll
-            for (int it = 0; it < NIT; ++it) {
-                const int g = min(it * (HF_NW * 8) + (tid >> 3), NG - 1), y0 = p0 - r + 8 * g;
-#pragma unroll
-                for (int e = 0; e < 8; ++e) ld[it][e] = *reinterpret_cast<const hf_f32x4 *>(src + (long)clampi(y0 + e, 0, Y - 1) * X + xq);
-            }
-        } else {
-#pragma unroll
-            for (int it = 0; it < NIT; ++it) {
-                const int g = min(it * (HF_NW * 8) + (tid >> 3), NG - 1), y0 = p0 - r + 8 * g;
-#pragma unroll
-                for (int e = 0; e < 8; ++e) {
-                    const float *row = src + (long)clampi(y0 + e, 0, Y - 1) * X;
-                    ld[it][e] = hf_f32x4{row[min(xq, X - 1)], row[min(xq + 1, X - 1)], row[min(xq + 2, X - 1)], row[min(xq + 3, X - 1)]};
-                }
-            }
-        }
-#pragma unroll
-        for (int it = 0; it < NIT; ++it) {
-            const int g = it * (HF_NW * 8) + (tid >> 3);
-            if (g < NG) {
-                float v[8];
-#pragma unroll
-                for (int e = 0; e < 8; ++e) v[e] = ld[it][e].x;
-                split8(v, 4 * lq, g);
-#pragma unroll
-                for (int e = 0; e < 8; ++e) v[e] = ld[it][e].y;
-                split8(v, 4 * lq + 1, g);
-#pragma unroll
-                for (int e = 0; e < 8; ++e) v[e] = ld[it][e].z;
-                split8(v, 4 * lq + 2, g);
-#pragma unroll
-                for (int e = 0; e < 8; ++e) v[e] = ld[it][e].w;
-                split8(v, 4 * lq + 3, g);
-            }
-        }
-    }
-    if (!(vmax < 40000.f)) atomicOr(range_flag, 8);
-    __syncthreads();
 
     const int i = lane & 31, h = lane >> 5;
     const int len = AXIS == 1 ? Y : X;
-    if (p0 + wave * 64 >= len) return;
+    const bool inside = p0 + wave * 64 < len;
     const _Float16 *bh = sB_hi + i * PITCH + wave * 64 + 8 * h, *bl = sB_lo + i * PITCH + wave * 64 + 8 * h;
     const int wrow0 = (h - (i >> 3) + 3) * 8 + (i & 7);
-    f32x16 thh[2], tm[2], ahh[2], am[2];
-#pragma unroll
-    for (int t = 0; t < 2; ++t)
-#pragma unroll
-        for (int q = 0; q < 16; ++q) { thh[t][q] = 0.f; tm[t][q] = 0.f; ahh[t][q] = 0.f; am[t][q] = 0.f; }
-    uint4 fh[3], fl[3];
     auto mm = [](const uint4 &wf, const uint4 &sf, const f32x16 &c) -> f32x16 {
         if (AXIS == 1) return __builtin_amdgcn_mfma_f32_32x32x16_f16(__builtin_bit_cast(f16x8, wf), __builtin_bit_cast(f16x8, sf), c, 0, 0, 0);
         return __builtin_amdgcn_mfma_f32_32x32x16_f16(__builtin_bit_cast(f16x8, sf), __builtin_bit_cast(f16x8, wf), c, 0, 0, 0);
     };
-    auto flush = [&](int t) {
+    auto flush = [](f32x16 &thh, f32x16 &tm, f32x16 &ahh, f32x16 &am) {
 #pragma unroll
         for (int q = 0; q < 16; q += 2) {
-            f32x2 x = f32x2{thh[t][q], thh[t][q + 1]} + f32x2{ahh[t][q], ahh[t][q + 1]};
-            f32x2 y = f32x2{tm[t][q], tm[t][q + 1]} + f32x2{am[t][q], am[t][q + 1]};
+            f32x2 x = f32x2{thh[q], thh[q + 1]} + f32x2{ahh[q], ahh[q + 1]};
+            f32x2 y = f32x2{tm[q], tm[q + 1]} + f32x2{am[q], am[q + 1]};
             asm volatile("" : "+v"(x), "+v"(y));
-            thh[t][q] = x[0]; thh[t][q + 1] = x[1];
-            tm[t][q] = y[0]; tm[t][q + 1] = y[1];
-            ahh[t][q] = 0.f; ahh[t][q + 1] = 0.f;
-            am[t][q] = 0.f; am[t][q + 1] = 0.f;
+            thh[q] = x[0]; thh[q + 1] = x[1];
+            tm[q] = y[0]; tm[q + 1] = y[1];
+            ahh[q] = 0.f; ahh[q + 1] = 0.f;
+            am[q] = 0.f; am[q + 1] = 0.f;
         }
     };
+    if constexpr (ARGMAX) {
+        const float dabs = cert_abs(clip_p95, clip_has);
+        CertTop top[2][16];
+#pragma unroll
+        for (int t = 0; t < 2; ++t)
+#pragma unroll
+            for (int q = 0; q < 16; ++q) top[t][q] = cert_start();
+        for (int z = 0; z < Z; ++z) {
+            if (z) __syncthreads();
+            stage(in + (long)z * P);
+            __syncthreads();
+            if (!inside) continue;
+#pragma unroll
+            for (int t = 0; t < 2; ++t) {
+                f32x16 thh, tm, ahh, am;
+#pragma unroll
+                for (int q = 0; q < 16; ++q) { thh[q] = 0.f; tm[q] = 0.f; ahh[q] = 0.f; am[q] = 0.f; }
+                uint4 sh = *reinterpret_cast<const uint4 *>(bh + 32 * t), sl = *reinterpret_cast<const uint4 *>(bl + 32 * t);
+#pragma unroll
+                for (int s = 0; s < S; ++s) {
+                    const uint4 wh = sW_hi[wrow0 + 16 * s], wl = sW_lo[wrow0 + 16 * s];
+                    uint4 nsh = sh, nsl = sl;
+                    if (s + 1 < S) {
+                        nsh = *reinterpret_cast<const uint4 *>(bh + 16 * (s + 1 + 2 * t));
+                        nsl = *reinterpret_cast<const uint4 *>(bl + 16 * (s + 1 + 2 * t));
+                    }
+                    ahh = mm(wh, sh, ahh);
+                    am = mm(wh, sl, am);
+                    am = mm(wl, sh, am);
+                    if ((s & 1) == 1 || s == S - 1) flush(thh, tm, ahh, am);
+                    __builtin_amdgcn_sched_barrier(0);
+                    sh = nsh; sl = nsl;
+                }
+#pragma unroll
+                for (int q = 0; q < 16; ++q)
+                    cert_push(top[t][q], __builtin_fmaf(tm[q], 4.8828125e-4f, thh[q]) * sc.inv, z, dabs);
+            }
+        }
+        if (inside) {
+#pragma unroll
+            for (int t = 0; t < 2; ++t) {
+                const int xx = p0 + wave * 64 + 32 * t + i;
+#pragma unroll
+                for (int q = 0; q < 16; ++q) {
+                    const int yy = l0 + (q & 3) + 8 * (q >> 2) + 4 * h;
+                    if (yy >= Y || xx >= X) continue;
+                    top_b[(long)yy * X + xx] = float2{top[t][q].b1, top[t][q].b2};
+                    top_z[(long)yy * X + xx] = top[t][q].zz;
+                }
+            }
+        }
+        return;
+    }
+    stage(in + (long)blockIdx.y * P);
+    __syncthreads();
+    if (!inside) return;
+    f32x16 thh[2], tm[2], ahh[2], am[2];
+#pragma unroll
+    for (int t = 0; t < 2; ++t)
+#pragma unroll
+        for (int q = 0; q < 16; ++q) { thh[t][q] = 0.f; tm[t][q] = 0.f; ahh[t][q] = 0.f; am[t][q] = 0.f; }
+    uint4 fh[3], fl[3];
 #pragma unroll
     for (int s = 0; s < S + 2; ++s) {
         const uint4 sh = *reinterpret_cast<const uint4 *>(bh + 16 * s), sl = *reinterpret_cast<const uint4 *>(bl + 16 * s);
@@ -196,18 +290,18 @@
             ahh[0] = mm(fh[s % 3], sh, ahh[0]);
             am[0] = mm(fh[s % 3], sl, am[0]);
             am[0] = mm(fl[s % 3], sh, am[0]);
-            if ((s & 1) == 1 || s == S - 1) flush(0);
+            if ((s & 1) == 1 || s == S - 1) flush(thh[0], tm[0], ahh[0], am[0]);
         }
         if (s >= 2) {
             const int k = (s - 2) % 3;
             ahh[1] = mm(fh[k], sh, ahh[1]);
             am[1] = mm(fh[k], sl, am[1]);
             am[1] = mm(fl[k], sh, am[1]);
-            if (((s - 2) & 1) == 1 || s == S + 1) flush(1);
+            if (((s - 2) & 1) == 1 || s == S + 1) flush(thh[1], tm[1], ahh[1], am[1]);
         }
         __builtin_amdgcn_sched_barrier(0);
     }
-    float *dst = out + (long)z * P;
+    float *dst = out + (long)blockIdx.y * P;
 #pragma unroll
     for (int t = 0; t < 2; ++t) {
         const int o0 = p0 + wave * 64 + 32 * t;
diff --git a/tissue_image_processing_amd/csrc/tip_internal.h b/tissue_image_processing_amd/csrc/tip_internal.h
--- a/tissue_image_processing_amd/csrc/tip_internal.h
+++ b/tissue_image_processing_amd/csrc/tip_internal.h
@@ -104,6 +104,7 @@
     int ws_no_endgame = 0, ws_no_wide = 0;
     int project_generic = 0, project_unfused_preblur = 0, project_unfused_mask = 0;
     int project_exact_score = 0, project_debug = 0;
+    int argmax_fused = 1;
     int unet_tail_unfused = 0;
     int unet_xcd_map = 1;
     int unet_spb = 3;
diff --git a/tissue_image_processing_amd/csrc/tip_project.hip b/tissue_image_processing_amd/csrc/tip_project.hip
--- a/tissue_image_processing_amd/csrc/tip_project.hip
+++ b/tissue_image_processing_amd/csrc/tip_project.hip
@@ -7,6 +7,7 @@
 #include <algorithm>
 #include <atomic>
 #include <cstdlib>
+#include <vector>
 
 namespace tip {
 
@@ -15,16 +16,6 @@
     float p95;
     int has;
 };
-
-template <typename T>
-__device__ __forceinline__ T wave_inclusive_scan(T v, int lane)
-{
-    for (int d = 1; d < 64; d <<= 1) {
-        const T o = __shfl_up(v, d, 64);
-        if (lane >= d) v += o;
-    }
-    return v;
-}
 
 constexpr int HIST_PER_BLOCK = 57344;
 __device__ __forceinline__ void hist_clear(unsigned int *h)
@@ -372,46 +363,52 @@
     return f;
 }
 
-template <int AXIS>
-static int launch_f16(const float *in, float *out, int Zs, int Y, int X, const TapsF &t, const ClipInfo *clip, int *range_flag)
+constexpr int ARGMAX_MAX_Z = 32;
+template <int AXIS, bool ARGMAX = false>
+static int launch_f16(const float *in, float *out, int Zs, int Y, int X, const TapsF &t, const ClipInfo *clip, int *range_flag,
+                      float2 *top_b = nullptr, unsigned *top_z = nullptr)
 {
     if (t.n != 241 || !clip || !range_flag) return fail(TIP_ERR_ARG, "f16 score pass: %d taps (241 only) or no clip value / range flag", t.n);
+    if (ARGMAX && (Zs > ARGMAX_MAX_Z || !top_b || !top_z))
+        return fail(TIP_ERR_ARG, "f16 score pass with argmax: %d planes (at most %d) or no buffers", Zs, ARGMAX_MAX_Z);
     constexpr int R8 = 15, NPOS = HF_TO + 16 * R8, PITCH = ((NPOS / 8) | 1) * 8, WROWS = 2 * (R8 + 2) + 3;
     const size_t lds = (size_t)2 * HF_LN * PITCH * 2 + (size_t)2 * WROWS * 8 * 16;
-    auto k = k_corr_long_f16<AXIS, R8>;
+    auto k = k_corr_long_f16<AXIS, R8, ARGMAX>;
     static std::atomic<unsigned> attr_done[64];
     const int dev = ctx().device >= 0 && ctx().device < 64 ? ctx().device : 0;
-    if (!(attr_done[dev].load(std::memory_order_acquire) & (1u << AXIS))) {
+    constexpr unsigned bit = 1u << (AXIS + (ARGMAX ? 2 : 0));
+    if (!(attr_done[dev].load(std::memory_order_acquire) & bit)) {
         TIP_HIP(hipFuncSetAttribute((const void *)k, hipFuncAttributeMaxDynamicSharedMemorySize, (int)lds));
-        attr_done[dev].fetch_or(1u << AXIS, std::memory_order_release);
+        attr_done[dev].fetch_or(bit, std::memory_order_release);
     }
     const int tiles_ln = cdiv(AXIS == 1 ? X : Y, HF_LN), tiles_pos = cdiv(AXIS == 1 ? Y : X, HF_TO);
     if ((long)tiles_ln * tiles_pos > 0x7fffffffL || Zs > 65535) return fail(TIP_ERR_ARG, "f16 score pass: grid too large");
-    const dim3 grid((unsigned)(tiles_ln * tiles_pos), (unsigned)Zs);
+    const dim3 grid((unsigned)(tiles_ln * tiles_pos), ARGMAX ? 1u : (unsigned)Zs);
     const int xcd_bands = (AXIS == 2 && tiles_ln % 8 == 0) ? 1 : 0;
     TIP_LAUNCH(AXIS == 1 ? "score_fast_y" : "score_fast_x", k, grid, dim3(HF_NW * 64), lds, in, out, Zs, Y, X, t, &clip->p95, &clip->has, range_flag,
-               tiles_ln, tiles_pos, xcd_bands);
-    return TIP_OK;
-}
-
-#define CERT_EPS (96.0f * 5.9604644775390625e-8f)
-__device__ __forceinline__ float cert_abs(const ClipInfo *clip)
-{
-    return (clip && clip->has) ? clip->p95 * 5.684341886080802e-14f + 1e-30f : 1e-30f;
-}
-
+               tiles_ln, tiles_pos, xcd_bands, top_b, top_z);
+    return TIP_OK;
+}
+
+
+template <bool TOPS>
 __global__ void __launch_bounds__(256) k_argmax_certify(const float *__restrict__ score, int Z, long P, int *__restrict__ best_z,
-                                                        int *__restrict__ unc_list, int *__restrict__ unc_count, const ClipInfo *clip)
+                                                        int *__restrict__ unc_list, unsigned long long *__restrict__ unc_planes,
+                                                        int *__restrict__ unc_count, const ClipInfo *clip,
+                                                        const float2 *__restrict__ top_b, const unsigned *__restrict__ top_z)
 {
     __shared__ int s_cnt[4], s_base;
-    const float dabs = cert_abs(clip);
+    const float dabs = cert_abs(&clip->p95, &clip->has);
     const long p0 = ((long)blockIdx.x * blockDim.x + threadIdx.x) * 4;
     const bool vec = p0 + 4 <= P && (P & 3) == 0;
-    float b1[4], b2[4];
-    int z1[4];
-#pragma unroll
-    for (int k = 0; k < 4; ++k) { b1[k] = -1.f; b2[k] = -1.f; z1[k] = 0; }
-    if (p0 < P) {
+    CertTop top[4];
+#pragma unroll
+    for (int k = 0; k < 4; ++k) top[k] = cert_start();
+    if (TOPS) {
+#pragma unroll
+        for (int k = 0; k < 4; ++k)
+            if (p0 + k < P) top[k] = CertTop{top_b[p0 + k].x, top_b[p0 + k].y, top_z[p0 + k]};
+    } else if (p0 < P) {
         for (int z = 0; z < Z; ++z) {
             float v[4];
             if (vec) {
@@ -422,19 +419,15 @@
                 for (int k = 0; k < 4; ++k) v[k] = p0 + k < P ? score[(long)z * P + p0 + k] : 0.f;
             }
 #pragma unroll
-            for (int k = 0; k < 4; ++k) {
-                if (v[k] > b1[k]) { b2[k] = b1[k]; b1[k] = v[k]; z1[k] = z; }
-                else if (v[k] > b2[k]) b2[k] = v[k];
-            }
+            for (int k = 0; k < 4; ++k) cert_push(top[k], v[k], z, dabs);
         }
     }
     unsigned unc = 0;
 #pragma unroll
     for (int k = 0; k < 4; ++k) {
         if (p0 + k >= P) continue;
-        best_z[p0 + k] = z1[k];
-        const bool certain = (b1[k] == 0.f) || (Z == 1) || (b1[k] * (1.f - CERT_EPS) - dabs > b2[k] * (1.f + CERT_EPS) + dabs);
-        if (!certain) unc |= 1u << k;
+        best_z[p0 + k] = cert_best(top[k]);
+        if (!cert_certain(top[k], Z, dabs)) unc |= 1u << k;
     }
     const int mine = __popc(unc);
     const int lane = threadIdx.x & 63, wave = threadIdx.x >> 6;
@@ -451,65 +444,86 @@
         for (int w = 0; w < wave; ++w) off += s_cnt[w];
 #pragma unroll
         for (int k = 0; k < 4; ++k)
-            if ((unc >> k) & 1u) unc_list[off++] = (int)(p0 + k);
-    }
-}
-
-constexpr int FIX_UL = 16;
-__global__ void __launch_bounds__(256) k_argmax_exact_fix(const float *__restrict__ zvol, const float *__restrict__ score, int Z, int Y,
-                                                          int X, Taps taps, const int *__restrict__ unc_list,
-                                                          const int *__restrict__ unc_count, int *__restrict__ best_z, const ClipInfo *clip)
-{
-    const float dabs = cert_abs(clip);
+            if ((unc >> k) & 1u) {
+                unc_list[off] = (int)(p0 + k);
+                unc_planes[off++] = cert_planes(top[k], Z);
+            }
+    }
+}
+
+constexpr int FIX_UL = 16, FIX_W = 16;
+__global__ void __launch_bounds__(256) k_argmax_exact_fix(const float *__restrict__ zvol, int Z, int Y, int X, Taps taps,
+                                                          const int *__restrict__ unc_list, const unsigned long long *__restrict__ unc_planes,
+                                                          const int *__restrict__ unc_count, int *__restrict__ best_z)
+{
     __shared__ float c[256];
-    __shared__ float sfast[64];
-    __shared__ float sexact[64];
-    __shared__ int s_z;
-    const int r = taps.n >> 1;
+    __shared__ int s_p[64], s_n;
+    __shared__ unsigned long long s_m[64];
+    const int r = taps.n >> 1, tid = threadIdx.x;
+    const int wlog = 2 * r + FIX_W <= 256 ? 4 : 0;
+    static_assert(FIX_W == 16, "wlog");
+    const long P = (long)Y * X;
     const int total = *unc_count, xcd = blockIdx.x & 7, per = (total + 7) / 8;
     for (int sl = blockIdx.x >> 3; sl < per; sl += gridDim.x >> 3) {
         const int u = xcd * per + sl;
         if (u >= total) break;
-        const int p = unc_list[u];
-        const int y = p / X, x = p - y * X;
-        const long P = (long)Y * X;
-        if (threadIdx.x < Z) sfast[threadIdx.x] = score[(long)threadIdx.x * P + p];
+        const int p = unc_list[u], before = unc_list[max(u - 1, 0)];
+        const int y = p / X, cell = (p - y * X) >> wlog, x0 = cell << wlog;
+        auto in_cell = [&](int q) { const int qy = q / X; return qy == y && ((q - qy * X) >> wlog) == cell; };
+        if (u > 0 && in_cell(before)) continue;
         __syncthreads();
-        float smax = sfast[0];
-        for (int z = 1; z < Z; ++z) smax = fmaxf(smax, sfast[z]);
-        const float thr = smax * (1.f - CERT_EPS) - dabs;
+        if (tid < 64) {
+            const bool have = u + tid < total;
+            const int q = have ? unc_list[u + tid] : -1;
+            const unsigned long long m = have ? unc_planes[u + tid] : 0ULL;
+            const unsigned long long same = __ballot(have && in_cell(q));
+            const int n = ~same ? __ffsll((unsigned long long)~same) - 1 : 64;
+            if (tid < n) { s_p[tid] = q; s_m[tid] = m; }
+            if (tid == 0) s_n = n;
+        }
+        __syncthreads();
+        const int n = s_n;
+        unsigned long long planes = 0ULL;
+        int lo = FIX_W, hi = 0;
+        for (int k = 0; k < n; ++k) {
+            const int dxk = s_p[k] - y * X - x0;
+            planes |= s_m[k];
+            lo = min(lo, dxk);
+            hi = max(hi, dxk);
+        }
+        const bool own = tid < n;
+        const int dx = own ? s_p[tid] - y * X - x0 : 0;
+        const unsigned long long mine = own ? s_m[tid] : 0ULL;
+        float b = -2.f;
+        int bz = 0;
         for (int z = 0; z < Z; ++z) {
-            const bool cand = sfast[z] * (1.f + CERT_EPS) + dabs >= thr;
-            if (!cand) { if (threadIdx.x == 0) sexact[z] = -1.f; continue; }
+            if (!((planes >> z) & 1ULL)) continue;
             const float *vol = zvol + (long)z * P;
-            if (threadIdx.x < 2 * r + 1) {
-                const int xx = clampi(x + (int)threadIdx.x - r, 0, X - 1);
+            if (tid >= lo && tid <= hi + 2 * r) {
+                const int xx = clampi(x0 - r + tid, 0, X - 1);
                 double tmp = (double)vol[(long)y * X + xx] * taps.w[r];
                 for (int d0 = r; d0 >= 1; d0 -= FIX_UL) {
-                    float a[FIX_UL], b[FIX_UL];
-#pragma unroll
-                    for (int u = 0; u < FIX_UL; ++u) {
-                        const int d = max(d0 - u, 1);
-                        a[u] = vol[(long)clampi(y - d, 0, Y - 1) * X + xx];
-                        b[u] = vol[(long)clampi(y + d, 0, Y - 1) * X + xx];
+                    float va[FIX_UL], vb[FIX_UL];
+#pragma unroll
+                    for (int k = 0; k < FIX_UL; ++k) {
+                        const int d = max(d0 - k, 1);
+                        va[k] = vol[(long)clampi(y - d, 0, Y - 1) * X + xx];
+                        vb[k] = vol[(long)clampi(y + d, 0, Y - 1) * X + xx];
                     }
 #pragma unroll
-                    for (int u = 0; u < FIX_UL; ++u)
-                        if (d0 - u >= 1) tmp += ((double)a[u] + (double)b[u]) * taps.w[r - (d0 - u)];
+                    for (int k = 0; k < FIX_UL; ++k)
+                        if (d0 - k >= 1) tmp += ((double)va[k] + (double)vb[k]) * taps.w[r - (d0 - k)];
                 }
-                c[threadIdx.x] = (float)tmp;
+                c[tid] = (float)tmp;
             }
             __syncthreads();
-            if (threadIdx.x == 0) sexact[z] = (float)tap_sum(r, [&](int j) { return (double)c[j]; }, taps.w);
+            if ((mine >> z) & 1ULL) {
+                const float e = (float)tap_sum(r, [&](int j) { return (double)c[dx + j]; }, taps.w);
+                if (e > b) { b = e; bz = z; }
+            }
             __syncthreads();
         }
-        if (threadIdx.x == 0) {
-            float b = -2.f; int bz = 0;
-            for (int z = 0; z < Z; ++z)
-                if (sexact[z] > b) { b = sexact[z]; bz = z; }
-            best_z[p] = bz;
-        }
-        __syncthreads();
+        if (own) best_z[s_p[tid]] = bz;
     }
 }
 
@@ -690,25 +704,40 @@
 {
     const int Zs = s.Zs, Y = s.Y, X = s.X;
     const long P = s.P;
-    float *D = s.ws.get<float>(s.V);
+    const bool fused = Zs <= ARGMAX_MAX_Z && tuning().argmax_fused;
+    float *D = fused ? nullptr : s.ws.get<float>(s.V);
+    float2 *topb = fused ? s.ws.get<float2>(P) : nullptr;
+    unsigned *topz = fused ? s.ws.get<unsigned>(P) : nullptr;
     int *bestz = s.ws.get<int>(P), *unc = s.ws.get<int>(P), *uncn = s.ws.get<int>(1);
-    if (!D || !bestz || !unc || !uncn) return TIP_ERR_NOMEM;
+    unsigned long long *uncp = s.ws.get<unsigned long long>(P);
+    if ((fused ? !topb || !topz : !D) || !bestz || !unc || !uncp || !uncn) return TIP_ERR_NOMEM;
     const TapsF f30 = taps_f32(s.k30.w, s.k30.n);
     int rc;
     if ((rc = launch_f16<1>((const float *)s.B, s.A, Zs, Y, X, f30, s.clip, s.err))) return rc;
-    if ((rc = launch_f16<2>((const float *)s.A, D, Zs, Y, X, f30, s.clip, s.err))) return rc;
     TIP_HIP(hipMemsetAsync(uncn, 0, sizeof(int), s.stream));
-    TIP_LAUNCH("argmax_certify", k_argmax_certify, dim3(cdiv(cdiv(P, 4), 256)), dim3(256), 0, (const float *)D, Zs, P, bestz, unc, uncn,
-               (const ClipInfo *)s.clip);
-    TIP_LAUNCH("argmax_exact_fix", k_argmax_exact_fix, dim3(8192), dim3(256), 0, (const float *)s.B, (const float *)D, Zs, Y, X,
-               s.k30, (const int *)unc, (const int *)uncn, bestz, (const ClipInfo *)s.clip);
+    if (fused) {
+        if ((rc = launch_f16<2, true>((const float *)s.A, nullptr, Zs, Y, X, f30, s.clip, s.err, topb, topz))) return rc;
+        TIP_LAUNCH("argmax_certify", k_argmax_certify<true>, dim3(cdiv(cdiv(P, 4), 256)), dim3(256), 0, (const float *)nullptr, Zs, P, bestz, unc,
+                   uncp, uncn, (const ClipInfo *)s.clip, (const float2 *)topb, (const unsigned *)topz);
+    } else {
+        if ((rc = launch_f16<2>((const float *)s.A, D, Zs, Y, X, f30, s.clip, s.err))) return rc;
+        TIP_LAUNCH("argmax_certify", k_argmax_certify<false>, dim3(cdiv(cdiv(P, 4), 256)), dim3(256), 0, (const float *)D, Zs, P, bestz, unc,
+                   uncp, uncn, (const ClipInfo *)s.clip, (const float2 *)nullptr, (const unsigned *)nullptr);
+    }
+    TIP_LAUNCH("argmax_exact_fix", k_argmax_exact_fix, dim3(8192), dim3(256), 0, (const float *)s.B, Zs, Y, X, s.k30, (const int *)unc,
+               (const unsigned long long *)uncp, (const int *)uncn, bestz);
     if ((rc = emit_from_planes(s, bestz, s.min_z))) return rc;
     if (tuning().project_debug) {
         int hn = 0, he = 0;
         TIP_HIP(hipMemcpyAsync(&hn, uncn, sizeof(int), hipMemcpyDeviceToHost, s.stream));
         TIP_HIP(hipMemcpyAsync(&he, s.err, sizeof(int), hipMemcpyDeviceToHost, s.stream));
         TIP_HIP(hipStreamSynchronize(s.stream));
-        fprintf(stderr, "certified argmax: %d of %ld pixels recomputed exactly\n", hn, P);
+        std::vector<unsigned long long> hp((size_t)hn);
+        if (hn) TIP_HIP(hipMemcpy(hp.data(), uncp, (size_t)hn * sizeof(unsigned long long), hipMemcpyDeviceToHost));
+        long two = 0, all = 0;
+        for (unsigned long long m : hp) (__builtin_popcountll(m) <= 2 ? two : all)++;
+        fprintf(stderr, "certified argmax: %d of %ld pixels recomputed exactly (%s; %ld with two candidate planes, %ld with all %d)\n", hn, P,
+                fused ? "argmax in the x pass" : "argmax over the score volume", two, all, Zs);
         if (he & 8) return fail(TIP_ERR_HIP, "score pass: a sample beyond the clip value's range reached the fp16 tiles");
     }
     return TIP_OK;
```
